# wengroup/matten

Hardware: AMD Instinct MI355X
Metric: edge_tensor_products_per_sec (higher is better)
Workload: dtype f32; 1 GPU; configs[2]: synthetic fcc-64 crystals (64 atoms, cutoff 5 A, 1152 edges each), paper hparams lmax=4, eval forward backbone+out_layer, one batch per step per GPU; last conv layer run for its live outputs only (258/842 radial-weight columns: the irreps its only reader takes) -- `value` counts 4 edge-TP per edge all the same, `value_full_layers` is the rate with the full last layer; nodes_per_gpu=64000, edges_per_gpu=1152000, conv_layers=4

## Files before the change

### include/matten_hip.h

```cpp
#ifndef MATTEN_HIP_H
#define MATTEN_HIP_H

#include <stddef.h>
#include <stdint.h>

#ifdef __cplusplus
extern "C" {
#endif

typedef void* matten_stream_t;

#define MATTEN_OK 0
#define MATTEN_EINVAL (-1)
#define MATTEN_ELAUNCH (-2)
#define MATTEN_ENOMEM (-3)

int matten_abi_version(void);

#define MATTEN_RADIAL_MAX_MID 3

size_t matten_csr_workspace_bytes(int64_t n_edges, int64_t n_nodes);
int matten_csr_counting_max_avg_degree(void);
int matten_csr_build(const int64_t* edge_index, int64_t n_edges, int64_t n_nodes, int32_t* perm,
                     int32_t* rowptr, int32_t* src_sorted, void* workspace, size_t workspace_bytes,
                     int32_t* err_flag, matten_stream_t stream);

int64_t matten_csr_split_bound(int64_t n_nodes, int64_t n_edges, int64_t max_len);
int matten_csr_split(const int32_t* rowptr, int64_t n_nodes, int64_t n_edges, int64_t max_len, int32_t* vrowptr,
                     int64_t* vseg, const float* num_neigh, float* vnn, matten_stream_t stream);

size_t matten_group_workspace_bytes(int64_t n, int64_t n_keys);
int matten_group_by_key(const int64_t* key, int64_t n, int64_t n_keys, int32_t* order, int32_t* seg,
                        void* workspace, size_t workspace_bytes, int32_t* err_flag, matten_stream_t stream);

int matten_species_embed(const int64_t* atomic_numbers, int64_t n_nodes, const int64_t* z_to_index,
                         int64_t min_z, int64_t max_z, int64_t n_species, const float* weight ,
                         const float* bias , int64_t dim, int64_t* species_index, int32_t* species_i32,
                         float* node_feats, float* node_attrs, int32_t* err_flag, matten_stream_t stream);

int matten_edge_geom(const float* pos, const int64_t* edge_index, const float* edge_cell_shift,
                     const float* cell, int64_t n_cells, const int64_t* batch, const int32_t* perm,
                     int64_t n_edges, int64_t n_nodes, int lmax, int n_basis, float r_start, float r_end,
                     float* geom_sorted, float* sh_sorted, int sh_stride, float* edge_vectors, float* edge_lengths,
                     float* edge_attrs, float* edge_embedding, matten_stream_t stream);
int matten_edge_geom_bwd(const float* geom_sorted, const float* dy, int64_t sh_stride, const float* dlen, int lmax,
                         int64_t n_edges, int64_t n_nodes, const int32_t* rowptr, const int32_t* out_ptr,
                         const int32_t* out_perm, const int32_t* perm, const float* edge_cell_shift, int64_t n_cells,
                         const int64_t* ptr, float* dv, float* dpos, float* dcell, matten_stream_t stream);

int matten_radial_mlp(const float* geom_sorted, int64_t n_edges, int n_basis, float r_start, float r_end,
                      const float* w0p, int nb_pad, const float* w1p, const float* w2p, int hidden, int w_pad,
                      float act_cst, void* w_edge, int out_is_bf16, matten_stream_t stream);
int matten_radial_mlp_deep(const float* geom_sorted, int64_t n_edges, int n_basis, float r_start, float r_end,
                           const float* w0p, int nb_pad, const float* w_mid, int n_mid, const float* w2p, int hidden,
                           int w_pad, float act_cst, void* w_edge, int out_is_bf16, matten_stream_t stream);

int matten_tp_tile_nodes(void);
int matten_tp_paths(const float* x, int64_t d_in, const void* w_edge, int64_t w_pad, const float* sh_sorted,
                    int64_t sh_dim, const int32_t* rowptr, const int32_t* src_sorted, int64_t n_nodes,
                    const int32_t* path_entries, const int32_t* unit_start, int64_t n_entries,
                    int64_t units_per_tile, int64_t d_mid, float avg_num_neighbors, const float* num_neigh,
                    float* agg , int w_is_bf16, matten_stream_t stream);

int matten_agg_linear_max_mt(void);
int matten_agg_linear_block_chunks(void);
size_t matten_agg_linear_lds_bytes(int64_t w_stride, int64_t n_io, int64_t n_blocks);
size_t matten_agg_linear_max_lds_bytes(void);
int matten_agg_linear(const float* agg, int64_t ld, const int32_t* order, const int32_t* seg, int64_t n_species,
                      const float* wtab, int64_t w_stride, const int32_t* io_table, int64_t n_io,
                      const int32_t* blocks, int64_t n_blocks, const float* add, int64_t add_ld, int64_t d_out,
                      int64_t n_rows, float* out, matten_stream_t stream);
int matten_agg_linear_gate(const float* agg, int64_t ld, const int32_t* order, const int32_t* seg, int64_t n_species,
                           const float* wtab, int64_t w_stride, const int32_t* io_table, int64_t n_io,
                           const int32_t* blocks, int64_t n_blocks, const float* add, int64_t add_ld, int64_t d_out,
                           int64_t n_rows, const int32_t* cmeta, const float* act_cst, const float* bn_scale,
                           const float* bn_shift, int64_t d_act, float* out, matten_stream_t stream);
int matten_agg_linear_gate_sets(void);
int matten_radial_hidden(const float* geom_sorted, int64_t n_edges, int n_basis, float r_start, float r_end,
                         const float* w0p, int nb_pad, const float* w1p, int hidden, uint16_t* h2s,
                         const float* h_scale, matten_stream_t stream);
int matten_radial_hidden_multi(const float* geom_sorted, int64_t n_edges, int n_basis, float r_start, float r_end,
                               const float* const* w0p, int nb_pad, const float* const* w1p, int hidden,
                               uint16_t* const* h2s, const float* const* h_scale, int n_layers,
                               matten_stream_t stream);
int matten_radial_hidden_deep(const float* geom_sorted, int64_t n_edges, int n_basis, float r_start, float r_end,
                              const float* w0p, int nb_pad, const float* w_mid, int n_mid, int hidden, uint16_t* h2s,
                              const float* h_scale, matten_stream_t stream);
int matten_radial_hidden_multi_deep(const float* geom_sorted, int64_t n_edges, int n_basis, float r_start, float r_end,
                                    const float* const* w0p, int nb_pad, const float* const* w_mid, int n_mid, int hidden,
                                    uint16_t* const* h2s, const float* const* h_scale, int n_layers,
                                    matten_stream_t stream);
int matten_tp_fused(const float* x, int64_t d_in, const uint16_t* h2s, const float* w2p, int64_t w_pad,
                    const float* sh_sorted, int64_t sh_stride, const int32_t* rowptr, const int32_t* src_sorted,
                    int64_t n_nodes, const int32_t* group_entries, const int32_t* unit_map, int64_t n_entries,
                    int64_t units_per_tile, int64_t lds_floats_per_wave, int64_t d_mid, float avg_num_neighbors,
                    const float* num_neigh, const uint16_t* a_split, const float* a_scale_inv,
                    float* agg , matten_stream_t stream);

int matten_tp_wreg(void);
int matten_tp_max_cols(void);
int matten_tp_max_cols_l0(void);
int matten_tp_max_cols_l1(void);
int matten_tp_groups_hash(void);

int matten_species_linear(const float* x, int64_t d_in, const int32_t* order, const int32_t* seg, int64_t n_species,
                          const float* wp, int64_t w_stride, const int32_t* segs, int64_t n_segs, int64_t d_out,
                          const float* add, int64_t add_ld, int64_t n_rows, float* out, matten_stream_t stream);

int matten_species_linear_rows(const float* x, int64_t d_in, const int32_t* order, const int32_t* seg, int64_t n_species,
                               const float* wp, int64_t w_stride, const int32_t* segs, int64_t n_segs, int64_t d_out,
                               const float* add, int64_t add_ld, int64_t n_rows, float* out, matten_stream_t stream);

int matten_species_linear_walk_all_blocks(void);
int64_t matten_species_linear_lds_w_floats(void);
int64_t matten_species_linear_rows_lds_bytes(void);

int matten_gate_bn(const float* x, int64_t d_in, const int32_t* meta, int64_t d_out, const float* act_cst,
                   const float* running_mean, const float* running_var, const float* bn_weight,
                   const float* bn_bias, float eps, int64_t n_rows, float* out, matten_stream_t stream);

int matten_segment_reduce(const float* x, int64_t dim, const int64_t* ptr, int64_t n_segments, int mean,
                          float* out, matten_stream_t stream);
int matten_segment_minmax(const float* x, int64_t dim, const int64_t* ptr, int64_t n_segments, int take_max, float* out,
                          int64_t* arg, matten_stream_t stream);
int matten_segment_minmax_bwd(const float* dy, int64_t dim, const int64_t* arg, int64_t n_segments, float* dx,
                              matten_stream_t stream);

int64_t matten_radial_mlp_bwd_small_slices(int64_t n_edges);
int64_t matten_radial_mlp_bwd_w2_ranges(int64_t n_edges, int64_t w_pad);
int matten_radial_mlp_bwd(const float* geom_sorted, int64_t n_edges, int n_basis, float r_start, float r_end,
                          const float* w0p, int nb_pad, const float* w1p, const float* w2p, int hidden, int w_pad,
                          int w_cols, const void* dw, int64_t dw_ld, int dw_is_bf16, float* h2_scratch,
                          float* part_small, float* part_w2, float scale0, float scale1, float scale2,
                          float* grad_small, float* grad_w2, matten_stream_t stream);
int64_t matten_radial_mlp_bwd_w2_ranges_deep(int64_t n_edges, int64_t w_pad, int n_mid);
int matten_radial_mlp_bwd_deep(const float* geom_sorted, int64_t n_edges, int n_basis, float r_start, float r_end,
                               const float* w0p, int nb_pad, const float* w_mid, int n_mid, const float* w2p, int hidden,
                               int w_pad, int w_cols, const void* dw, int64_t dw_ld, int dw_is_bf16, float* h2_scratch,
                               float* part_small, float* part_w2, float scale0, float scale1, float scale2,
                               float* grad_small, float* grad_w2, matten_stream_t stream);
int matten_radial_mlp_bwd_len(const float* geom_sorted, int64_t n_edges, int n_basis, float r_start, float r_end,
                              const float* w0p, int nb_pad, const float* w_mid, int n_mid, const float* w2p, int hidden,
                              int w_pad, int w_cols, const void* dw, int64_t dw_ld, int dw_is_bf16, float* dlen,
                              matten_stream_t stream);
int matten_radial_pack(const float* w0, const float* w1, const float* w2, int n_basis, int nb_pad, int w_cols, int w_pad,
                       float scale0, float scale1, float scale2, float* w0p, float* w1p, float* w2p,
                       matten_stream_t stream);
int matten_radial_pack_deep(const float* w0, const float* w_mid, int n_mid, const float* w2, int n_basis, int nb_pad,
                            int w_cols, int w_pad, float scale0, float scale1, float scale2, float* w0p, float* w_mid_p,
                            float* w2p, matten_stream_t stream);
int matten_radial_pack_cols(const float* w0, const float* w1, const float* w2, int n_basis, int nb_pad, int w_cols,
                            const int64_t* cols, int n_cols, int w_pad, float scale0, float scale1, float scale2, float* w0p,
                            float* w1p, float* w2p, matten_stream_t stream);
int matten_radial_h_scale(const float* w0, const float* w1, int n_basis, float r_start, float r_end, float act_cst,
                          float* out2, matten_stream_t stream);
int matten_radial_pack_cols_deep(const float* w0, const float* w_mid, int n_mid, const float* w2, int n_basis, int nb_pad,
                                 int w_cols, const int64_t* cols, int n_cols, int w_pad, float scale0, float scale1,
                                 float scale2, float* w0p, float* w_mid_p, float* w2p, matten_stream_t stream);
int matten_radial_h_scale_deep(const float* w0, const float* w_mid, int n_mid, int n_basis, float r_start, float r_end,
                               float act_cst, float* out2, matten_stream_t stream);
int matten_split_a_tiles(const float* w2p, int64_t w_pad, const int32_t* group_entries, int64_t n_entries,
                         const float* h_scale, uint16_t* frag, float* scale_inv, matten_stream_t stream);
int matten_gather_scale(const float* src, const int64_t* idx, const float* scale, int64_t n, int64_t scale_period,
                        int scale_by_source, float* out, const int64_t* perm2, float* out2, matten_stream_t stream);
int64_t matten_species_linear_wgrad_scratch_floats(int64_t n_rows, int64_t n_species, int64_t w_stride);

int matten_dense_rows(const float* x, int64_t n_in, const float* q, int64_t n_out, int64_t n_rows, float* out,
                      matten_stream_t stream);

int matten_elastic_props(const void* c, int is_fp64, int layout, int64_t n, double* voigt, double* compliance,
                         double* props, int32_t* flags, matten_stream_t stream);
int matten_elastic_props_bwd(const double* voigt, const double* compliance, const double* props, const int32_t* flags,
                             const double* g_props, const double* g_voigt, const double* g_compliance, int is_fp64,
                             int layout, int64_t n, void* g_c, matten_stream_t stream);
int matten_elastic_directional(const double* compliance, const int32_t* flags, const double* dirs, int64_t n,
                               int64_t n_dirs, double* young, double* beta, double* ext, int32_t* arg,
                               matten_stream_t stream);
int matten_elastic_pair(const double* compliance, const int32_t* flags, const double* dirs, const double* cos_sin,
                        int64_t n, int64_t n_dirs, int64_t n_angles, double* maps, double* ext, int32_t* arg,
                        matten_stream_t stream);
int matten_elastic_acoustic(const double* voigt, const int32_t* flags, const double* density, const double* dirs, int64_t n,
                            int64_t n_dirs, double modulus_unit, double* vel, double* ext, int32_t* arg, int32_t* n_unstable,
                            matten_stream_t stream);
int matten_elastic_directional_bwd(const double* compliance, const int32_t* flags, const double* dirs, int64_t n,
                                   int64_t n_dirs, const double* g_young, const double* g_beta, const double* g_ext,
                                   const int32_t* arg, double* g_compliance, matten_stream_t stream);
int matten_elastic_acoustic_bwd(const double* voigt, const int32_t* flags, const double* density, const double* dirs,
                                int64_t n, int64_t n_dirs, double modulus_unit, const double* g_vel, const double* g_ext,
                                const int32_t* arg, double* g_voigt, matten_stream_t stream);
int matten_elastic_refine(const double* compliance, const int32_t* flags, const double* dirs, const double* cos_sin,
                          const double* ext_dir, const int32_t* arg_dir, const double* ext_pair, const int32_t* arg_pair,
                          int64_t n, int64_t n_dirs, int64_t n_angles, double tol, int64_t max_iter, double* value,
                          double* vec_n, double* vec_m, int32_t* status, int32_t* iterations, matten_stream_t stream);

int matten_elastic_kelvin(const double* voigt, const int32_t* flags, int64_t n, double* moduli, double* vectors,
                          double* dilatation, matten_stream_t stream);
int matten_elastic_kelvin_bwd(const double* vectors, const int32_t* flags, const double* g_moduli, int64_t n,
                              double* g_voigt, matten_stream_t stream);
int matten_elastic_kelvin_clamp(const double* voigt, const double* moduli, const double* vectors, double floor, int64_t n,
                                double* out, matten_stream_t stream);

int matten_elastic_polycrystal(const double* voigt, const int32_t* flags, const double* moduli, const double* vectors,
                               int64_t n, int hs_grid, double sc_tol, int sc_max_iter, double* out, double* media,
                               int32_t* status, matten_stream_t stream);
int matten_elastic_polycrystal_bwd(const double* voigt, const int32_t* flags, const double* out, const int32_t* status,
                                   const double* g_sc, int64_t n, double* g_voigt, matten_stream_t stream);

int matten_rank2_props(const void* t, int is_fp64, int64_t n, double* vals, double* axes, double* props, int32_t* flags,
                       matten_stream_t stream);
int matten_rank2_props_bwd(const double* vals, const double* axes, const double* props, const int32_t* flags,
                           const double* g_vals, const double* g_props, int is_fp64, int64_t n, void* g_t,
                           matten_stream_t stream);

int matten_wigner_d(const double* R, int64_t G, int lmax, double orth_tol, double* D, int32_t* flags, matten_stream_t stream);
int matten_irreps_rotate(const void* x, int is_fp64, int64_t n, int64_t dim, const int32_t* layout, int K, const double* D,
                         const int32_t* flags, const int32_t* index, int64_t G, int transpose, void* out,
                         matten_stream_t stream);
int matten_irreps_average(const void* x, int is_fp64, int64_t n, int64_t dim, const int32_t* layout, int K, const double* D,
                          const int32_t* flags, int64_t G, const int64_t* op_ptr, const int32_t* op_idx,
                          const double* weights, int transpose, void* out, double* deviation, matten_stream_t stream);

#define MATTEN_SYM_MAX_OPS 48
#define MATTEN_SYM_MAX_ATOMS 1024
#define MATTEN_SYM_NOT_FINITE 1
#define MATTEN_SYM_RANGE 2
#define MATTEN_SYM_TOO_LARGE 4
#define MATTEN_SYM_AMBIGUOUS 8
#define MATTEN_SYM_TRUNC 16
#define MATTEN_SYM_NOT_PERIODIC 32
int matten_lattice_group(const double* cell, int64_t B, double symprec, int8_t* N_out, int32_t* n_lat, int32_t* flags,
                         matten_stream_t stream);
int matten_crystal_symmetry(const double* pos, const double* cell, const int64_t* Z, const int64_t* ptr, const uint8_t* pbc,
                            int64_t B, int64_t N_total, double symprec, int max_trans, const int8_t* N_in,
                            const int32_t* n_lat, const int32_t* lat_flags, double* rot, int8_t* rot_int, double* trans,
                            int32_t* n_rot, int32_t* src, int32_t* n_trans, double* ttrans, int32_t* tsrc, int32_t* flags,
                            matten_stream_t stream);
int matten_irreps_average_atoms(const void* x, int is_fp64, int64_t n, int64_t dim, const int32_t* layout, int K,
                                const double* D, const int32_t* flags, int64_t B, int64_t G_cap, const int32_t* n_ops,
                                const int32_t* row_struct, const int32_t* src, void* out, matten_stream_t stream);



int matten_tp_backward(const float* x, int64_t d_in, const void* w_edge, int64_t w_ld, const float* sh_sorted,
                       int64_t sh_stride, const int32_t* src_sorted, const int32_t* dst_sorted,
                       const int32_t* col_meta, int64_t n_cols, const uint8_t* nnz_ijk, const float* nnz_c,
                       const float* g_agg, int64_t d_mid, float avg_num_neighbors, const float* num_neigh,
                       int64_t n_edges, float* dx, void* dw, int64_t dw_ld, const int32_t* in_ptr,
                       const int32_t* in_cols, int64_t n_in, int edge_is_bf16 ,
                       matten_stream_t stream);

// ... 187 lines not shown
```

### matten_amd/_lib.py

```python
from __future__ import annotations

import ctypes
import os
from ctypes import c_float, c_int, c_int32, c_int64, c_size_t, c_void_p

_HERE = os.path.dirname(os.path.abspath(__file__))
LIB_PATH = os.path.join(_HERE, "libmatten_hip.so")

ABI_VERSION = 47

P = c_void_p
SIGNATURES = {
    "matten_abi_version": (c_int, []),
    "matten_csr_workspace_bytes": (c_size_t, [c_int64, c_int64]),
    "matten_group_workspace_bytes": (c_size_t, [c_int64, c_int64]),
    "matten_csr_counting_max_avg_degree": (c_int, []),
    "matten_csr_build": (c_int, [P, c_int64, c_int64, P, P, P, P, c_size_t, P, P]),
    "matten_csr_split_bound": (c_int64, [c_int64, c_int64, c_int64]),
    "matten_csr_split": (c_int, [P, c_int64, c_int64, c_int64, P, P, P, P, P]),
    "matten_group_by_key": (c_int, [P, c_int64, c_int64, P, P, P, c_size_t, P, P]),
    "matten_species_embed": (c_int, [P, c_int64, P, c_int64, c_int64, c_int64, P, P, c_int64, P, P, P, P, P, P]),
    "matten_edge_geom": (c_int, [P, P, P, P, c_int64, P, P, c_int64, c_int64, c_int, c_int, c_float, c_float, P, P, c_int, P, P, P, P, P]),
    "matten_radial_mlp": (c_int, [P, c_int64, c_int, c_float, c_float, P, c_int, P, P, c_int, c_int, c_float, P, c_int, P]),
    "matten_radial_mlp_deep": (c_int, [P, c_int64, c_int, c_float, c_float, P, c_int, P, c_int, P, c_int, c_int, c_float, P, c_int,
                                       P]),
    "matten_tp_tile_nodes": (c_int, []),
    "matten_tp_paths": (c_int, [P, c_int64, P, c_int64, P, c_int64, P, P, c_int64, P, P, c_int64, c_int64, c_int64, c_float, P, P, c_int,
                                P]),
    "matten_radial_hidden_multi": (c_int, [P, c_int64, c_int, c_float, c_float, P, c_int, P, c_int, P, P, c_int, P]),
    "matten_radial_hidden_multi_deep": (c_int, [P, c_int64, c_int, c_float, c_float, P, c_int, P, c_int, c_int, P, P, c_int, P]),
    "matten_agg_linear_max_mt": (c_int, []),
    "matten_agg_linear_block_chunks": (c_int, []),
    "matten_agg_linear_lds_bytes": (c_size_t, [c_int64, c_int64, c_int64]),
    "matten_agg_linear_max_lds_bytes": (c_size_t, []),
    "matten_agg_linear": (c_int, [P, c_int64, P, P, c_int64, P, c_int64, P, c_int64, P, c_int64, P, c_int64, c_int64,
                                  c_int64, P, P]),
    "matten_agg_linear_gate": (c_int, [P, c_int64, P, P, c_int64, P, c_int64, P, c_int64, P, c_int64, P, c_int64, c_int64,
                                       c_int64, P, P, P, P, c_int64, P, P]),
    "matten_agg_linear_gate_sets": (c_int, []),
    "matten_radial_hidden": (c_int, [P, c_int64, c_int, c_float, c_float, P, c_int, P, c_int, P, P, P]),
    "matten_radial_hidden_deep": (c_int, [P, c_int64, c_int, c_float, c_float, P, c_int, P, c_int, c_int, P, P, P]),
    "matten_tp_wreg": (c_int, []),
    "matten_tp_max_cols": (c_int, []),
    "matten_tp_max_cols_l0": (c_int, []),
    "matten_tp_max_cols_l1": (c_int, []),
    "matten_tp_groups_hash": (c_int, []),
    "matten_tp_fused": (c_int, [P, c_int64, P, P, c_int64, P, c_int64, P, P, c_int64, P, P, c_int64, c_int64, c_int64, c_int64, c_float, P, P, P, P, P]),
    "matten_species_linear": (c_int, [P, c_int64, P, P, c_int64, P, c_int64, P, c_int64, c_int64, P, c_int64, c_int64, P, P]),
    "matten_species_linear_rows": (c_int, [P, c_int64, P, P, c_int64, P, c_int64, P, c_int64, c_int64, P, c_int64, c_int64, P, P]),
    "matten_radial_mlp_bwd_small_slices": (c_int64, [c_int64]),
    "matten_radial_mlp_bwd_w2_ranges": (c_int64, [c_int64, c_int64]),
    "matten_radial_mlp_bwd_w2_ranges_deep": (c_int64, [c_int64, c_int64, c_int]),
    "matten_radial_mlp_bwd": (c_int, [P, c_int64, c_int, c_float, c_float, P, c_int, P, P, c_int, c_int, c_int, P, c_int64,
                                      c_int, P, P, P, c_float, c_float, c_float, P, P, P]),
    "matten_radial_mlp_bwd_deep": (c_int, [P, c_int64, c_int, c_float, c_float, P, c_int, P, c_int, P, c_int, c_int, c_int, P,
                                           c_int64, c_int, P, P, P, c_float, c_float, c_float, P, P, P]),
    "matten_radial_pack": (c_int, [P, P, P, c_int, c_int, c_int, c_int, c_float, c_float, c_float, P, P, P, P]),
    "matten_radial_pack_deep": (c_int, [P, P, c_int, P, c_int, c_int, c_int, c_int, c_float, c_float, c_float, P, P, P, P]),
    "matten_radial_pack_cols": (c_int, [P, P, P, c_int, c_int, c_int, P, c_int, c_int, c_float, c_float, c_float, P, P, P, P]),
    "matten_radial_pack_cols_deep": (c_int, [P, P, c_int, P, c_int, c_int, c_int, P, c_int, c_int, c_float, c_float, c_float, P, P,
                                             P, P]),
    "matten_radial_h_scale": (c_int, [P, P, c_int, c_float, c_float, c_float, P, P]),
    "matten_radial_h_scale_deep": (c_int, [P, P, c_int, c_int, c_float, c_float, c_float, P, P]),
    "matten_split_a_tiles": (c_int, [P, c_int64, P, c_int64, P, P, P, P]),
    "matten_gather_scale": (c_int, [P, P, P, c_int64, c_int64, c_int, P, P, P, P]),
    "matten_species_linear_walk_all_blocks": (c_int, []),
    "matten_species_linear_lds_w_floats": (c_int64, []),
    "matten_species_linear_rows_lds_bytes": (c_int64, []),
    "matten_species_linear_wgrad_scratch_floats": (c_int64, [c_int64, c_int64, c_int64]),
    "matten_tp_backward": (c_int, [P, c_int64, P, c_int64, P, c_int64, P, P, P, c_int64, P, P, P, c_int64, c_float, P, c_int64, P, P, c_int64,
                                   P, P, c_int64, c_int, P]),
    "matten_tp_backward_lit": (c_int, [P, c_int64, P, c_int64, P, c_int64, P, P, P, c_int64, c_int64, P, c_int64, P, c_int64, c_float,
                                       P, c_int64, P, P, c_int64, c_int, c_int64, P, P, P, c_int, P]),
    "matten_tp_backward_lit_wfree": (c_int, [P, c_int64, P, P, P, P, c_int64, P, P, P, c_int64, c_int64, P, c_int64, P, c_int64, c_float,
                                             P, c_int64, P, P, c_int64, c_int, c_int64, P, P, P, c_int64, c_int, c_int, P]),
    "matten_tp_backward_sh": (c_int, [P, c_int64, P, c_int64, P, P, P, c_int64, c_int64, P, c_int64, P, c_int64, c_float, P, c_int64,
                                      c_int, P, c_int64, c_int, P]),
    "matten_radial_mlp_bwd_len": (c_int, [P, c_int64, c_int, c_float, c_float, P, c_int, P, c_int, P, c_int, c_int, c_int, P,
                                          c_int64, c_int, P, P]),
    "matten_edge_geom_bwd": (c_int, [P, P, c_int64, P, c_int, c_int64, c_int64, P, P, P, P, P, c_int64, P, P, P, P, P]),
    "matten_adam_step": (c_int, [P, P, P, P, c_int64, P, c_float, c_float, c_float, c_float, c_float, P]),
    "matten_adam_ctl_workspace_bytes": (c_size_t, [c_int64]),
    "matten_adam_step_ctl": (c_int, [P, P, P, P, P, c_int64, P, P, P, P, c_size_t, c_float, c_float, c_float, c_float, c_float,
                                     c_float, c_int, c_int, P]),
    "matten_species_linear_wgrad": (c_int, [P, c_int64, P, c_int64, P, P, c_int64, c_int64, P, c_int64, c_int64, P, P, P]),
    "matten_gate_bwd": (c_int, [P, c_int64, P, c_int64, P, P, c_int64, P, P]),
    "matten_bn_scratch_floats": (c_int64, [c_int64, c_int64]),
    "matten_bn_train_fwd": (c_int, [P, c_int64, c_int64, P, P, c_int64, P, P, c_float, P, P, P, P, P, c_float, P, P]),
    "matten_bn_train_bwd": (c_int, [P, P, c_int64, c_int64, P, P, c_int64, P, P, P, c_float, P, P, P, P, P, P, P]),
    "matten_bn_train_fwd_valid": (c_int, [P, c_int64, c_int64, P, P, c_int64, P, P, c_float, P, P, P, P, P, c_float, P, P, P]),
    "matten_bn_train_bwd_valid": (c_int, [P, P, c_int64, c_int64, P, P, c_int64, P, P, P, c_float, P, P, P, P, P, P, P, P]),
    "matten_norm_act": (c_int, [P, c_int64, c_int64, P, c_int64, c_int, c_float, P, P, P, P, c_float, P, P]),
    "matten_norm_act_bwd": (c_int, [P, P, c_int64, c_int64, P, c_int64, c_int, c_float, P, P]),
    "matten_bn_eval_bwd_scratch_floats": (c_int64, [c_int64, c_int64]),
    "matten_gate_bn_eval_bwd": (c_int, [P, c_int64, P, c_int64, P, P, c_int64, P, P, P, c_float, P, c_int64, P, P, P, P, P]),
    "matten_norm_act_bn_eval_bwd": (c_int, [P, P, c_int64, c_int64, P, c_int64, c_int, c_float, P, P, P, c_float, P, P, P, P,
                                            P]),
    "matten_instance_norm_fwd": (c_int, [P, c_int64, c_int64, P, P, c_int64, P, P, c_int64, P, P, c_float, P, P, P, P]),
    "matten_instance_norm_bwd": (c_int, [P, P, c_int64, c_int64, P, P, c_int64, P, P, c_int64, P, P, P, c_float, P, P, P, P]),
    "matten_segment_reduce_bwd": (c_int, [P, c_int64, P, c_int64, c_int, P, P]),
    "matten_graph_prep": (c_int, [P, P, P, c_int64, ctypes.c_double, P, P, P, P, P, P]),
    "matten_graph_prep_pbc": (c_int, [P, P, P, P, c_int64, ctypes.c_double, P, P, P, P, P, P, P, P]),
    "matten_neighbor_rows_count": (c_int, [P, P, P, P, P, P, ctypes.c_double, c_int64, P, P]),
    "matten_neighbor_rows_fill": (c_int, [P, P, P, P, P, P, ctypes.c_double, c_int64, P, c_int64, P, P, P, P]),
    "matten_neighbor_cells_row_capacity": (c_int, []),
    "matten_neighbor_cells_max_axis_bins": (c_int, []),
    "matten_neighbor_cells_grid": (c_int, [P, P, P, P, P, P, c_int64, ctypes.c_double, P, P, P, P]),
    "matten_neighbor_cells_bin": (c_int, [P, P, P, P, P, P, c_int64, P, P, P]),
    "matten_neighbor_cells_scatter": (c_int, [P, P, P, P, c_int64, P, P, P]),
    "matten_neighbor_cells_count": (c_int, [P, P, P, P, P, P, P, P, P, P, P, ctypes.c_double, c_int64, P, P]),
    "matten_neighbor_cells_fill": (c_int, [P, P, P, P, P, P, P, P, P, P, P, ctypes.c_double, c_int64, P, c_int64, P, P, P, P]),
    "matten_neighbor_count": (c_int, [P, P, P, P, P, P, ctypes.c_double, c_int64, c_int64, P, P, P]),
    "matten_neighbor_summary": (c_int, [P, P, c_int64, P, P]),
    "matten_neighbor_fill": (c_int, [P, P, P, P, P, P, ctypes.c_double, c_int64, c_int64, P, c_int64, P, P, P, P, c_int64,
                                     P, P, P, P]),
    "matten_neighbor_scan": (c_int, [P, c_int64, P, P]),
    "matten_neighbor_fill_capped": (c_int, [P, P, P, P, P, P, ctypes.c_double, c_int64, c_int64, P, P, c_int64, P, c_int64,
                                            c_int64, c_int64, P, P, P, P, P, P, P, P, P]),
    "matten_gate_bn": (c_int, [P, c_int64, P, c_int64, P, P, P, P, P, c_float, c_int64, P, P]),
    "matten_segment_reduce": (c_int, [P, c_int64, P, c_int64, c_int, P, P]),
    "matten_segment_minmax": (c_int, [P, c_int64, P, c_int64, c_int, P, P, P]),
    "matten_segment_minmax_bwd": (c_int, [P, c_int64, P, c_int64, P, P]),
    "matten_dense_rows": (c_int, [P, c_int64, P, c_int64, c_int64, P, P]),
    "matten_elastic_props": (c_int, [P, c_int, c_int, c_int64, P, P, P, P, P]),
    "matten_elastic_props_bwd": (c_int, [P, P, P, P, P, P, P, c_int, c_int, c_int64, P, P]),
    "matten_elastic_directional": (c_int, [P, P, P, c_int64, c_int64, P, P, P, P, P]),
    "matten_elastic_pair": (c_int, [P, P, P, P, c_int64, c_int64, c_int64, P, P, P, P]),
    "matten_elastic_acoustic": (c_int, [P, P, P, P, c_int64, c_int64, ctypes.c_double, P, P, P, P, P]),
    "matten_elastic_directional_bwd": (c_int, [P, P, P, c_int64, c_int64, P, P, P, P, P, P]),
    "matten_elastic_acoustic_bwd": (c_int, [P, P, P, P, c_int64, c_int64, ctypes.c_double, P, P, P, P, P]),
    "matten_elastic_refine": (c_int, [P, P, P, P, P, P, P, P, c_int64, c_int64, c_int64, ctypes.c_double, c_int64, P, P, P, P, P,
                                      P]),
    "matten_elastic_kelvin": (c_int, [P, P, c_int64, P, P, P, P]),
    "matten_elastic_kelvin_bwd": (c_int, [P, P, P, c_int64, P, P]),
    "matten_elastic_kelvin_clamp": (c_int, [P, P, P, ctypes.c_double, c_int64, P, P]),
    "matten_elastic_polycrystal": (c_int, [P, P, P, P, c_int64, c_int, ctypes.c_double, c_int, P, P, P, P]),
    "matten_elastic_polycrystal_bwd": (c_int, [P, P, P, P, P, c_int64, P, P]),
    "matten_rank2_props": (c_int, [P, c_int, c_int64, P, P, P, P, P]),
    "matten_rank2_props_bwd": (c_int, [P, P, P, P, P, P, c_int, c_int64, P, P]),
    "matten_wigner_d": (c_int, [P, c_int64, c_int, ctypes.c_double, P, P, P]),
    "matten_irreps_rotate": (c_int, [P, c_int, c_int64, c_int64, P, c_int, P, P, P, c_int64, c_int, P, P]),
    "matten_irreps_average": (c_int, [P, c_int, c_int64, c_int64, P, c_int, P, P, c_int64, P, P, P, c_int, P, P, P]),
    "matten_lattice_group": (c_int, [P, c_int64, ctypes.c_double, P, P, P, P]),
    "matten_crystal_symmetry": (c_int, [P, P, P, P, P, c_int64, c_int64, ctypes.c_double, c_int, P, P, P, P, P, P, P, P, P, P, P,
                                        P, P]),
    "matten_irreps_average_atoms": (c_int, [P, c_int, c_int64, c_int64, P, c_int, P, P, c_int64, c_int64, P, P, P, P, P]),
    "matten_batch_gather_lds_rows": (c_int, []),
    "matten_batch_gather_max_streams": (c_int, []),
    "matten_batch_gather": (c_int, [P, c_int64, P, c_int64, c_int64, c_int64, P]),
    "matten_batch_gather_padded": (c_int, [P, c_int64, P, c_int64, c_int64, c_int64, c_int64, c_int64, c_int64, P, P]),
    "matten_selected_loss_tile_elems": (c_int, []),
    "matten_selected_loss_max_blocks": (c_int, []),
    "matten_selected_loss_workspace_bytes": (c_size_t, [c_int64, c_int64]),
    "matten_selected_loss": (c_int, [P, P, P, c_int64, c_int64, c_int, P, P, P, P, c_size_t, P]),
    "matten_selected_loss_bwd": (c_int, [P, P, P, c_int64, c_int64, c_int, P, P, P, P]),
    "matten_valid_loss_workspace_bytes": (c_size_t, [c_int64, c_int64]),
    "matten_valid_loss": (c_int, [P, P, P, c_int64, c_int64, c_int, P, P, P, P, c_size_t, P]),
    "matten_valid_loss_bwd": (c_int, [P, P, P, c_int64, c_int64, c_int, P, P, P, P]),
}

_lib = None


class MattenHipError(RuntimeError):
    pass


def load() -> ctypes.CDLL:
    global _lib
    if _lib is not None:
        return _lib
    if not os.path.exists(LIB_PATH):
        raise MattenHipError(
            f"{LIB_PATH} not found: the HIP extension is not built. matten_amd has no CPU fallback; "
            "run `make -C matten_amd/csrc` (needs hipcc, --offload-arch=gfx950)."
        )
    import torch

    lib = ctypes.CDLL(LIB_PATH)
    for name, (res, args) in SIGNATURES.items():
        try:
            fn = getattr(lib, name)
        except AttributeError as e:
            raise MattenHipError(f"symbol {name} missing from {LIB_PATH}") from e
        fn.restype = res
        fn.argtypes = args
    v = lib.matten_abi_version()
    if v != ABI_VERSION:
        raise MattenHipError(f"ABI version mismatch: library {v}, python binding {ABI_VERSION}")
    _lib = lib
    return lib


_ERRORS = {-1: "MATTEN_EINVAL (bad argument)", -2: "MATTEN_ELAUNCH (HIP launch failed)", -3: "MATTEN_ENOMEM (workspace too small)"}


def check(rc: int, what: str) -> None:
    if rc != 0:
        raise MattenHipError(f"{what} failed: {_ERRORS.get(rc, rc)}")
```

### matten_amd/csrc/tp_fused.hip

```cpp
#include "tp_walk.h"

namespace {

using namespace matten_walk;

constexpr int KIND_MERGED = 256;
constexpr int KIND_WREG = 512;
struct StoreAgg {
    template <class G>
    __device__ __forceinline__ void store(const Args& a, const GroupEntry& ge, const float* __restrict__ acc,
                                          float a_scale_inv, int node, int j, int u, bool valid) const {
        if (TPF_LAB_NO_STORE ? (valid && acc[0] == 12345.678f) : valid) {
            const float nn = a.avg_nn > 0.0f ? a.avg_nn : a.num_neigh[node];
            const float norm = nn > 0.0f ? a_scale_inv / sqrtf(nn) : 0.0f;
            float* orow = a.agg + (int64_t)node * a.d_mid;
            const bool merged = (ge.kind & KIND_MERGED) != 0;
            const GroupEntry& g2 = (&ge)[merged ? 1 : 0];
            const bool second = merged && u >= 2;
            const unsigned mask = merged ? (second ? g2.mask : (unsigned)g2.w_base) : ge.mask;
            const int uc = second ? u - 2 : u;
#pragma unroll
            for (int cc = 0; cc < G::NC; ++cc) {
                if ((mask >> cc) & 1u) {
                    const int d3 = 2 * G::L3[cc] + 1;
                    const int ks = second ? g2.t_off[cc] : ge.t_off[cc];
                    float* op = orow + (second ? g2.out_off[cc] : ge.out_off[cc]) + (ks ? uc : uc * d3);
                    const int kstep = ks ? ks : 1;
#pragma unroll
                    for (int k = 0; k < 2 * matten::CG_LMAX + 1; ++k)
                        if (k < d3) op[k * kstep] = acc[G::OFF[cc] + k] * norm;
                }
            }
        }
    }
};

template <int L1, int GI>
__device__ __forceinline__ void run_group(const Args& a, const GroupEntry& ge, float* __restrict__ tile, int node,
                                          int lane, bool valid, int beg, int deg_node, int maxdeg) {
    const int deg = valid ? deg_node : 0;
    using G = matten::Group<L1, GI>;
    constexpr int NC = G::NC;
    float acc[G::NACC];
#pragma unroll
    for (int k = 0; k < G::NACC; ++k) acc[k] = 0.0f;

    const unsigned mask = ge.mask;
    const int cu_log2 = ge.cu_log2;
    const int cu = 1 << cu_log2;
    const int npw = 64 >> cu_log2;
    const int ch_log2 = npw >= 16 ? 0 : (4 - (6 - cu_log2));
    const int CH = 1 << ch_log2;
    const int T = npw >= 16 ? (npw >> 4) : 1;
    const int ncols = ge.mul * NC;
    const int MT = (ncols + 15) >> 4;
    const int ycol = MT * 16;
    const int stride = MT * 16 + 32 + 4;

    const int j = lane >> cu_log2;
    const int u = lane & (cu - 1);
    const int g = lane >> 4, c = lane & 15;
    const int xcol = ge.x_off + u * G::D1;
    const bool cmajor = WregOk<L1, GI, 3>::value && (ge.kind & KIND_WREG) != 0;
    const int wcol0 = cmajor ? u : u * NC, wstep = cmajor ? cu : 1;
    constexpr int CAPC = cap_channels(L1, NC);
    constexpr int MTMAX = (CAPC * NC + 15) / 16;
    f16x8 ah[MTMAX], al[MTMAX];
    float a_scale_inv;
    {
        float av[MTMAX][8];
        float amax = 0.0f;
#pragma unroll
        for (int mt = 0; mt < MTMAX; ++mt) {
#pragma unroll
            for (int kk = 0; kk < 8; ++kk) {
                const int k = 16 * (kk >> 2) + 4 * g + (kk & 3);
                av[mt][kk] = (mt < MT) ? a.w2p[(int64_t)k * a.w_pad + ge.w_base + mt * 16 + c] : 0.0f;
                amax = fmaxf(amax, fabsf(av[mt][kk]));
            }
        }
#pragma unroll
        for (int off = 32; off > 0; off >>= 1) amax = fmaxf(amax, __shfl_xor(amax, off));
        int e = (int)((__float_as_uint(amax) >> 23) & 0xffu) - 127;
        e = amax > 0.0f ? max(-100, min(100, e)) : 13;
        const float a_scale = __uint_as_float((unsigned)(127 + 13 - e) << 23);
        a_scale_inv = __uint_as_float((unsigned)(127 - 13 + e) << 23);
#pragma unroll
        for (int mt = 0; mt < MTMAX; ++mt) {
#pragma unroll
            for (int kk = 0; kk < 8; ++kk) {
                _Float16 hi, lo;
                split_f16(av[mt][kk] * a_scale, hi, lo);
                ah[mt][kk] = hi;
                al[mt][kk] = lo;
            }
        }
    }

    const int e_last = deg > 0 ? beg + deg - 1 : 0;
    float xn[G::D1];
    int src_nn;
    {
        const int src0 = a.src_sorted[min(beg, e_last)];
        src_nn = a.src_sorted[min(beg + 1, e_last)];
        const float* xp0 = a.x + (int64_t)src0 * a.d_in + xcol;
#pragma unroll
        for (int i = 0; i < G::D1; ++i) xn[i] = xp0[i];
    }
    for (int s0 = 0; s0 < maxdeg; s0 += CH) {
#pragma unroll
        for (int t = 0; t < 4; ++t) {
            if (t < T) {
                const int n = 16 * t + c;
                const int jn = n >> ch_log2, so = n & (CH - 1);
                const int begn = __shfl(beg, jn << cu_log2);
                const int degn = __shfl(deg_node, jn << cu_log2);
                f16x8 bh = {0, 0, 0, 0, 0, 0, 0, 0}, bl = {0, 0, 0, 0, 0, 0, 0, 0};
                if (s0 + so < degn) {
                    const int64_t en = begn + s0 + so;
                    const f16x8* hp = reinterpret_cast<const f16x8*>(a.h2s + en * (2 * HID) + g * 8);
                    bh = hp[0];
                    bl = hp[HID / 8];
                    const f32x4* yp4 = reinterpret_cast<const f32x4*>(a.sh + en * a.sh_stride + g * 8);
                    f32x4* yd = reinterpret_cast<f32x4*>(tile + (16 * t + c) * stride + ycol + g * 8);
                    yd[0] = yp4[0];
                    yd[1] = yp4[1];
                }
#pragma unroll
                for (int mt = 0; mt < MTMAX; ++mt) {
                    if (mt < MT) {
                        const f32x4 zero = {0.f, 0.f, 0.f, 0.f};
                        f32x4 dx = __builtin_amdgcn_mfma_f32_16x16x32_f16(al[mt], bh, zero, 0, 0, 0);
                        f32x4 dh = __builtin_amdgcn_mfma_f32_16x16x32_f16(ah[mt], bh, zero, 0, 0, 0);
                        dx = __builtin_amdgcn_mfma_f32_16x16x32_f16(ah[mt], bl, dx, 0, 0, 0);
                        *reinterpret_cast<f32x4*>(tile + (16 * t + c) * stride + mt * 16 + 4 * g) =
                            dh + SPLIT_LO_INV * dx;
                    }
                }
            }
        }
        __builtin_amdgcn_s_waitcnt(0xc07f);
        __builtin_amdgcn_wave_barrier();
        for (int so = 0; so < CH; ++so) {
            const int s = s0 + so;
            if (s >= maxdeg) break;
            float x[G::D1];
#pragma unroll
            for (int i = 0; i < G::D1; ++i) x[i] = xn[i];
            {
                const float* xp = a.x + (int64_t)src_nn * a.d_in + xcol;
#pragma unroll
                for (int i = 0; i < G::D1; ++i) xn[i] = xp[i];
                src_nn = a.src_sorted[min(beg + s + 2, e_last)];
            }
            if (s < deg) {
                const float* wp = tile + ((j << ch_log2) + so) * stride + wcol0;
                const float* yp = tile + ((j << ch_log2) + so) * stride + ycol + G::Y0;
                float y[G::NY], w[NC];
#pragma unroll
                for (int jj = 0; jj < G::NY; ++jj) y[jj] = yp[jj];
#pragma unroll
                for (int cc = 0; cc < NC; ++cc) w[cc] = wp[cc * wstep];
                G::apply(mask, x, y, w, acc);
            }
        }
        __builtin_amdgcn_wave_barrier();
    }
    StoreAgg{}.store<G>(a, ge, acc, a_scale_inv, node, j, u, valid);
}

#define MATTEN_RGS_ARGS a, ge, tile, stage, (um >> 8) & 0xffff, tile_id, r, reps, lane, StoreAgg{}
#define MATTEN_RGS_WR(L1, GI, TT, TD, P, WR) \
    do { \
        using HM = HotMask<L1, GI>; \
        if (HM::M0 && ge.mask == HM::M0) run_group_shared<L1, GI, TT, TD, P, HM::M0, WR>(MATTEN_RGS_ARGS); \
        else if (HM::M1 && ge.mask == HM::M1) run_group_shared<L1, GI, TT, TD, P, HM::M1, WR>(MATTEN_RGS_ARGS); \
        else run_group_shared<L1, GI, TT, TD, P, 0u, WR>(MATTEN_RGS_ARGS); \
    } while (0)
template <int L1, int GI, int TT, int TD, bool P>
__device__ __forceinline__ void run_group_shared_any(const Args& a, const GroupEntry& ge, float* __restrict__ tile,
                                                     float* __restrict__ stage, int um, int tile_id, int r, int reps, int lane) {
    if constexpr (TT == 1 && WregOk<L1, GI, 4>::value) {
        if ((ge.kind & KIND_WREG) && ge.cu_log2 == 4) {
            MATTEN_RGS_WR(L1, GI, TT, TD, P, 4);
            return;
        }
    }
    if constexpr (TT == 1 && WregOk<L1, GI, 3>::value) {
        if ((ge.kind & KIND_WREG) && ge.cu_log2 == 3) {
            MATTEN_RGS_WR(L1, GI, TT, TD, P, 3);
            return;
        }
    }
    if (ge.kind & KIND_WREG) return;
    MATTEN_RGS_WR(L1, GI, TT, TD, P, 0);
}
#define MATTEN_RGS(L1, GI, TT, TD, P) run_group_shared_any<L1, GI, TT, TD, P>(a, ge, tile, stage, um, tile_id, r, reps, lane)
#if defined(MATTEN_LAB) && defined(TPF_ONLY_VARIANT)
#ifndef TPF_ONLY_MASK
#define TPF_ONLY_MASK 0
#endif
#ifndef TPF_ONLY_WR
#define TPF_ONLY_WR 0
#endif
#define MATTEN_RGS_ONLY(L1, GI, TT, TD, P) run_group_shared<L1, GI, TT, TD, P, (unsigned)(TPF_ONLY_MASK), (TT == 1 ? TPF_ONLY_WR : 0)>(MATTEN_RGS_ARGS)
#define MATTEN_GROUP_CASE_SHARED(L1, GI) \
    case (L1 * matten::GROUP_KIND_STRIDE + GI): \
        if (TPF_ONLY_VARIANT == 0) MATTEN_RGS_ONLY(L1, GI, 1, (TPF_CHUNK_DEEP && L1 == 0 ? 2 : 0), true); \
        else if (TPF_ONLY_VARIANT == 1) MATTEN_RGS_ONLY(L1, GI, 2, 0, false); \
        else if (TPF_ONLY_VARIANT == 2) MATTEN_RGS_ONLY(L1, GI, 1, (TPF_CHUNK_DEEP && L1 == 0 ? 2 : TwoDeepOk<L1, GI>::value ? 1 : 0), false); \
        else MATTEN_RGS_ONLY(L1, GI, 1, 0, false); \
        break;
#else
#define MATTEN_GROUP_CASE_SHARED(L1, GI) \
    case (L1 * matten::GROUP_KIND_STRIDE + GI): \
        if (paired && TPF_CHUNK_DEEP && L1 == 0 && nodes_per_wave <= 8 && nodes_per_wave >= 4) MATTEN_RGS(L1, GI, 1, (L1 == 0 ? 2 : 0), true); \
        else if (paired) MATTEN_RGS(L1, GI, 1, 0, true); \
        else if (nodes_per_wave > 16) MATTEN_RGS(L1, GI, 2, 0, false); \
        else if (TPF_CHUNK_DEEP && L1 == 0 && nodes_per_wave <= 8 && nodes_per_wave >= 4) MATTEN_RGS(L1, GI, 1, (L1 == 0 ? 2 : 0), false); \
        else if (TwoDeepOk<L1, GI>::value && nodes_per_wave <= 8 && nodes_per_wave >= TPF_TWO_DEEP_MIN_NPW) MATTEN_RGS(L1, GI, 1, (TwoDeepOk<L1, GI>::value ? 1 : 0), false); \
        else MATTEN_RGS(L1, GI, 1, 0, false); \
        break;
#endif

#define MATTEN_GROUP_CASE(L1, GI) \
    case (L1 * matten::GROUP_KIND_STRIDE + GI): run_group<L1, GI>(a, ge, tile, un.node, lane, un.valid, un.beg, un.deg, un.maxdeg); break;

#ifndef TPF_MIN_BLOCKS
#define TPF_MIN_BLOCKS 3
#endif
#ifndef TPF_CHUNK_DEEP
#define TPF_CHUNK_DEEP 1
#endif
#ifndef TPF_TWO_DEEP_MIN_NPW
#define TPF_TWO_DEEP_MIN_NPW 2
#endif
#if defined(MATTEN_LAB) && defined(TPF_ONLY_L1) && defined(TPF_ONLY_GI)
#define TPF_FOR_EACH_GROUP(X) X(TPF_ONLY_L1, TPF_ONLY_GI)
#elif defined(MATTEN_LAB) && defined(TPF_ONLY_LIGHT)
#define TPF_FOR_EACH_GROUP(X) X(0, 0) X(1, 0) X(1, 1)
#elif defined(MATTEN_LAB) && defined(TPF_ONLY_HEAVY)
#define TPF_FOR_EACH_GROUP(X) X(2, 0) X(2, 1) X(3, 0) X(3, 1) X(4, 0) X(4, 1)
#else
#define TPF_FOR_EACH_GROUP(X) MATTEN_FOR_EACH_GROUP(X)
#endif
__global__ __launch_bounds__(WAVES_PER_BLOCK * 64, TPF_MIN_BLOCKS) void tp_fused_kernel(Args a, const GroupEntry* __restrict__ entries,
                                                                        const int* __restrict__ umap,
                                                                        int n_entries, int units_per_tile,
                                                                        int blocks_per_tile, int n_tiles) {
    extern __shared__ __attribute__((aligned(16))) float lds[];
    const int xcd = blockIdx.x % N_XCD;
    const int q = blockIdx.x / N_XCD;
    const int tile_id = (q / blocks_per_tile) * N_XCD + xcd;
    if (tile_id >= n_tiles) return;
    const int wave = __builtin_amdgcn_readfirstlane(threadIdx.x >> 6);
    const int unit = (q % blocks_per_tile) * WAVES_PER_BLOCK + wave;
    if (unit >= units_per_tile) return;
    const int lane = threadIdx.x & 63;
    float* tile = lds + wave * a.lds_per_wave;

    const int um = __builtin_amdgcn_readfirstlane(umap[unit]);
    if (((um >> 8) & 0xffff) >= n_entries) return;
    const GroupEntry& ge = entries[(um >> 8) & 0xffff];
    const int r = um & 255;
    const bool shared_stage = (um >> 24) & 1;
    const int reps = 1 << ((um >> 27) & 3);

    const int cu_log2 = ge.cu_log2;
    const int nodes_per_wave = 64 >> cu_log2;
    if (shared_stage) {
        float* stage = lds + WAVES_PER_BLOCK * a.lds_per_wave;
        const bool paired = (um >> 26) & 1;
        if ((um >> 25) & 1) {
            if (paired) run_loader_only_paired(a, ge, stage, tile_id, r, reps, lane);
            else run_loader_only(a, ge, stage, tile_id, r, reps, lane);
            return;
        }
        switch (ge.kind & (KIND_MERGED - 1)) {
            TPF_FOR_EACH_GROUP(MATTEN_GROUP_CASE_SHARED)
            default: break;
        }
        return;
    }
#if !(defined(MATTEN_LAB) && defined(TPF_ONLY_VARIANT))
    const UnitNodes un = unit_nodes(a, ge, tile_id, r, lane);
    switch (ge.kind & (KIND_MERGED - 1)) {
        TPF_FOR_EACH_GROUP(MATTEN_GROUP_CASE)
        default: break;
    }
#endif
}

constexpr int NT = 4;
__device__ __forceinline__ float silu(float z) {
#if defined(MATTEN_LAB) && defined(RH_ABLATE_NO_SILU)
    return z * 0.5f;
#endif
    return z * __builtin_amdgcn_rcpf(1.0f + __builtin_amdgcn_exp2f(-1.4426950408889634f * z));
}

template <int KS0, int N_MID>
__global__ __launch_bounds__(256) void radial_hidden_kernel(const float4* __restrict__ geom, int64_t E, int n_basis,
                                                            float r_start, float r_end,
                                                            const float* __restrict__ w0p,
                                                            const float* __restrict__ w_mid, _Float16* __restrict__ h2s,
                                                            const float* __restrict__ h_scale) {
    const int lane = threadIdx.x & 63;
    const int wave = threadIdx.x >> 6;
    const int g = lane >> 4, c = lane & 15;
    const int64_t e0 = ((int64_t)blockIdx.x * 4 + wave) * (NT * 16);
    if (e0 >= E) return;
    const float hs = h_scale ? *h_scale : 1.0f;
    const float inv_c = 1.0f / (r_end - r_start);
    const float bes_pref = sqrtf(2.0f * inv_c) * sqrtf((float)n_basis);
    float a1[N_MID > 0 ? N_MID : 1][2][8];
#pragma unroll
    for (int m = 0; m < N_MID; ++m)
#pragma unroll
        for (int kk = 0; kk < 8; ++kk) {
            int k = 16 * (kk >> 2) + 4 * g + (kk & 3);
            a1[m][0][kk] = w_mid[m * HID * HID + k * HID + c];
// ... 124 lines not shown
            }
#pragma unroll
            for (int r = 0; r < 4; ++r) {
                h0[r] = silu(h0[r]);
                h1[r] = silu(h1[r]);
            }
#pragma unroll
            for (int m = 0; m < N_MID; ++m) {
                f32x4 o0 = {0.f, 0.f, 0.f, 0.f}, o1 = {0.f, 0.f, 0.f, 0.f};
#pragma unroll
                for (int kk = 0; kk < 8; ++kk) {
                    const float b = kk < 4 ? h0[kk & 3] : h1[kk & 3];
                    o0 = __builtin_amdgcn_mfma_f32_16x16x4f32(a1[m][0][kk], b, o0, 0, 0, 0);
                    o1 = __builtin_amdgcn_mfma_f32_16x16x4f32(a1[m][1][kk], b, o1, 0, 0, 0);
                }
#pragma unroll
                for (int r = 0; r < 4; ++r) {
                    o0[r] = silu(o0[r]);
                    o1[r] = silu(o1[r]);
                }
                h0 = o0, h1 = o1;
            }
            if (e < E) {
                f16x8 hi, lo;
#pragma unroll
                for (int r = 0; r < 4; ++r) {
                    _Float16 h, ll;
                    split_f16(h0[r] * hs, h, ll);
                    hi[r] = h, lo[r] = ll;
                    split_f16(h1[r] * hs, h, ll);
                    hi[4 + r] = h, lo[4 + r] = ll;
                }
                f16x8* dst = reinterpret_cast<f16x8*>(h2s + e * (2 * HID) + g * 8);
                dst[0] = hi;
                dst[HID / 8] = lo;
            }
        }
    }
}

}

static int radial_hidden_multi_launch(const float* geom_sorted, int64_t n_edges, int n_basis, float r_start, float r_end,
                                      const float* const* w0p, int nb_pad, const float* const* w_mid, int n_mid, int hidden,
                                      uint16_t* const* h2s, const float* const* h_scale, int n_layers,
                                      matten_stream_t stream_) {
    hipStream_t stream = (hipStream_t)stream_;
    if (n_edges < 0 || hidden != HID || (nb_pad & 3) || nb_pad < n_basis || nb_pad > 16 || n_layers < 1 ||
        n_layers > RH_MAX_LAYERS || n_mid < 0 || n_mid > MATTEN_RADIAL_MAX_MID)
        return MATTEN_EINVAL;
    if (n_edges == 0) return MATTEN_OK;
    if (!geom_sorted || !w0p || (n_mid > 0 && !w_mid) || !h2s) return MATTEN_EINVAL;
    RadialLayers L{};
    L.n_layers = n_layers;
    for (int l = 0; l < n_layers; ++l) {
        if (!w0p[l] || (n_mid > 0 && !w_mid[l]) || !h2s[l]) return MATTEN_EINVAL;
        L.w0p[l] = w0p[l], L.w_mid[l] = n_mid > 0 ? w_mid[l] : nullptr, L.h2s[l] = (_Float16*)h2s[l];
        L.h_scale[l] = h_scale ? h_scale[l] : nullptr;
    }
    unsigned grid = (unsigned)matten_cdiv(n_edges, 4 * NT * 16);
#define LAUNCH(K, M) \
    radial_hidden_multi_kernel<K, M><<<grid, 256, 0, stream>>>((const float4*)geom_sorted, n_edges, n_basis, r_start, r_end, L)
#define LAUNCH_M(K)                  \
    switch (n_mid) {                 \
        case 0: LAUNCH(K, 0); break; \
        case 1: LAUNCH(K, 1); break; \
        case 2: LAUNCH(K, 2); break; \
        default: LAUNCH(K, 3); break; \
    }
    switch (nb_pad >> 2) {
        case 1: LAUNCH_M(1); break;
        case 2: LAUNCH_M(2); break;
        case 3: LAUNCH_M(3); break;
        default: LAUNCH_M(4); break;
    }
#undef LAUNCH_M
#undef LAUNCH
    MATTEN_LAUNCH_CHECK();
    return MATTEN_OK;
}

extern "C" int matten_radial_hidden_multi(const float* geom_sorted, int64_t n_edges, int n_basis, float r_start,
                                          float r_end, const float* const* w0p, int nb_pad, const float* const* w1p,
                                          int hidden, uint16_t* const* h2s, const float* const* h_scale, int n_layers,
                                          matten_stream_t stream_) {
    if (!w1p && n_edges > 0) return MATTEN_EINVAL;
    return radial_hidden_multi_launch(geom_sorted, n_edges, n_basis, r_start, r_end, w0p, nb_pad, w1p, 1, hidden, h2s,
                                      h_scale, n_layers, stream_);
}

extern "C" int matten_radial_hidden_multi_deep(const float* geom_sorted, int64_t n_edges, int n_basis, float r_start,
                                               float r_end, const float* const* w0p, int nb_pad, const float* const* w_mid,
                                               int n_mid, int hidden, uint16_t* const* h2s, const float* const* h_scale,
                                               int n_layers, matten_stream_t stream_) {
    return radial_hidden_multi_launch(geom_sorted, n_edges, n_basis, r_start, r_end, w0p, nb_pad, w_mid, n_mid, hidden, h2s,
                                      h_scale, n_layers, stream_);
}

static int radial_hidden_launch(const float* geom_sorted, int64_t n_edges, int n_basis, float r_start, float r_end,
                                const float* w0p, int nb_pad, const float* w_mid, int n_mid, int hidden, uint16_t* h2s,
                                const float* h_scale, matten_stream_t stream_) {
    hipStream_t stream = (hipStream_t)stream_;
    if (n_edges < 0 || hidden != HID || (nb_pad & 3) || nb_pad < n_basis || nb_pad > 16 || n_mid < 0 ||
        n_mid > MATTEN_RADIAL_MAX_MID)
        return MATTEN_EINVAL;
    if (n_edges == 0) return MATTEN_OK;
    if (!geom_sorted || !w0p || (n_mid > 0 && !w_mid) || !h2s) return MATTEN_EINVAL;
    unsigned grid = (unsigned)matten_cdiv(n_edges, 4 * NT * 16);
#define LAUNCH(K, M) \
    radial_hidden_kernel<K, M><<<grid, 256, 0, stream>>>((const float4*)geom_sorted, n_edges, n_basis, r_start, r_end, w0p, w_mid, (_Float16*)h2s, h_scale)
#define LAUNCH_M(K)                  \
    switch (n_mid) {                 \
        case 0: LAUNCH(K, 0); break; \
        case 1: LAUNCH(K, 1); break; \
        case 2: LAUNCH(K, 2); break; \
        default: LAUNCH(K, 3); break; \
    }
    switch (nb_pad >> 2) {
        case 1: LAUNCH_M(1); break;
        case 2: LAUNCH_M(2); break;
        case 3: LAUNCH_M(3); break;
        default: LAUNCH_M(4); break;
    }
#undef LAUNCH_M
#undef LAUNCH
    MATTEN_LAUNCH_CHECK();
    return MATTEN_OK;
}

extern "C" int matten_radial_hidden(const float* geom_sorted, int64_t n_edges, int n_basis, float r_start, float r_end,
                                    const float* w0p, int nb_pad, const float* w1p, int hidden, uint16_t* h2s,
                                    const float* h_scale, matten_stream_t stream_) {
    if (!w1p && n_edges > 0) return MATTEN_EINVAL;
    return radial_hidden_launch(geom_sorted, n_edges, n_basis, r_start, r_end, w0p, nb_pad, w1p, 1, hidden, h2s, h_scale,
                                stream_);
}

extern "C" int matten_radial_hidden_deep(const float* geom_sorted, int64_t n_edges, int n_basis, float r_start, float r_end,
                                         const float* w0p, int nb_pad, const float* w_mid, int n_mid, int hidden,
                                         uint16_t* h2s, const float* h_scale, matten_stream_t stream_) {
    return radial_hidden_launch(geom_sorted, n_edges, n_basis, r_start, r_end, w0p, nb_pad, w_mid, n_mid, hidden, h2s,
                                h_scale, stream_);
}

#if TPF_TRACING
static unsigned* g_tp_trace = nullptr;
static int64_t g_tp_trace_waves = 0, g_tp_trace_skip = 0;
extern "C" int matten_lab_tp_trace(unsigned* buf, int64_t n_waves, int64_t skip) {
    g_tp_trace = buf, g_tp_trace_waves = n_waves, g_tp_trace_skip = skip;
    return 0;
}
#endif

extern "C" int matten_tp_fused(const float* x, int64_t d_in, const uint16_t* h2s, const float* w2p, int64_t w_pad,
                               const float* sh_sorted, int64_t sh_stride, const int32_t* rowptr,
                               const int32_t* src_sorted, int64_t n_nodes, const int32_t* group_entries,
                               const int32_t* unit_map, int64_t n_entries, int64_t units_per_tile,
                               int64_t lds_floats_per_wave, int64_t d_mid, float avg_num_neighbors,
                               const float* num_neigh, const uint16_t* a_split, const float* a_scale_inv, float* agg,
                               matten_stream_t stream_) {
    hipStream_t stream = (hipStream_t)stream_;
    if (n_nodes < 0 || d_in <= 0 || w_pad <= 0 || sh_stride < 32 || (sh_stride & 3) || n_entries <= 0 ||
        units_per_tile <= 0 || d_mid <= 0 || lds_floats_per_wave <= 0 || (lds_floats_per_wave & 3))
        return MATTEN_EINVAL;
    if (n_nodes == 0) return MATTEN_OK;
    if (!x || !h2s || !w2p || !sh_sorted || !rowptr || !src_sorted || !group_entries || !unit_map || !agg)
        return MATTEN_EINVAL;
    if (!(avg_num_neighbors > 0.0f) && !num_neigh) return MATTEN_EINVAL;
    const size_t lds = sizeof(float) * ((size_t)lds_floats_per_wave * WAVES_PER_BLOCK + STAGE_TOTAL_FLOATS + PAIR_INFO_INTS);
    if (lds > 64 * 1024) return MATTEN_EINVAL;
    if ((a_split == nullptr) != (a_scale_inv == nullptr)) return MATTEN_EINVAL;
    Args a{x, (const _Float16*)h2s, w2p, (const _Float16*)a_split, a_scale_inv, sh_sorted, rowptr, src_sorted, num_neigh, agg, (int)d_in, (int)w_pad, (int)sh_stride,
           (int)d_mid, (int)n_nodes, (int)lds_floats_per_wave, avg_num_neighbors};
    const int n_tiles = (int)matten_cdiv(n_nodes, TILE_NODES);
    const int blocks_per_tile = (int)matten_cdiv(units_per_tile, WAVES_PER_BLOCK);
    const int64_t grid = matten_cdiv(n_tiles, N_XCD) * N_XCD * (int64_t)blocks_per_tile;
    if (grid >= ((int64_t)1 << 31)) return MATTEN_EINVAL;
#if TPF_TRACING
    a.trace = nullptr;
    if (g_tp_trace && grid * WAVES_PER_BLOCK <= g_tp_trace_waves) {
        if (g_tp_trace_skip <= 0) a.trace = g_tp_trace;
        if (g_tp_trace_skip == 0) g_tp_trace = nullptr;
        if (g_tp_trace_skip > 0) --g_tp_trace_skip;
    }
#endif
    tp_fused_kernel<<<(unsigned)grid, WAVES_PER_BLOCK * 64, lds, stream>>>(
        a, (const GroupEntry*)group_entries, unit_map, (int)n_entries, (int)units_per_tile, blocks_per_tile, n_tiles);
    MATTEN_LAUNCH_CHECK();
    return MATTEN_OK;
}

extern "C" int matten_tp_wreg(void) { return TPF_WREG ? TPF_WREG_MAX_L1 + 1 : 0; }
extern "C" int matten_tp_max_cols(void) { return TPF_MAX_COLS; }
extern "C" int matten_tp_max_cols_l0(void) { return TPF_MAX_COLS_L0; }
extern "C" int matten_tp_max_cols_l1(void) { return TPF_MAX_COLS_L1; }
extern "C" int matten_tp_groups_hash(void) { return matten::GROUPS_HASH; }
```

### matten_amd/csrc/tp_walk.h

```cpp
#pragma once
#include <type_traits>

#include "cg_gen.h"
#include "common.h"
#include "sh.h"

#ifndef MATTEN_LAB
#if defined(MATTEN_ABLATE_NO_GATHER) || defined(MATTEN_ABLATE_NO_XLOAD) || defined(MATTEN_ABLATE_NO_H2LOAD) || \
    defined(MATTEN_ABLATE_NO_MFMA) || defined(MATTEN_ABLATE_NO_VALU) || defined(MATTEN_ABLATE_NO_STORE) ||      \
    defined(MATTEN_ABLATE_NO_BARRIER) || defined(MATTEN_ABLATE_NO_LOOP) || defined(MATTEN_ABLATE_NO_EPI) || defined(MATTEN_ABLATE_ONE_YQUAD)
#error "MATTEN_ABLATE_* switches are honoured by -DMATTEN_LAB builds only (tools/*.sh)"
#endif
#endif
#if defined(MATTEN_LAB) && defined(MATTEN_ABLATE_NO_GATHER)
#define TPF_SRC(v) ((v) >= 0 ? (node < a.n_nodes ? node : 0) : 0)
#else
#define TPF_SRC(v) (v)
#endif
#if defined(MATTEN_LAB) && defined(MATTEN_ABLATE_NO_XLOAD)
#define TPF_XLD(xp, i, v) (1e-9f * (float)((v) + (i)))
#else
#define TPF_XLD(xp, i, v) ((xp)[i])
#endif
#if defined(MATTEN_LAB) && defined(MATTEN_ABLATE_NO_H2LOAD)
constexpr bool TPF_LAB_NO_H2LOAD = true;
#else
constexpr bool TPF_LAB_NO_H2LOAD = false;
#endif
#if defined(MATTEN_LAB) && defined(MATTEN_ABLATE_NO_MFMA)
constexpr bool TPF_LAB_NO_MFMA = true;
#else
constexpr bool TPF_LAB_NO_MFMA = false;
#endif
#if defined(MATTEN_LAB) && defined(MATTEN_ABLATE_NO_VALU)
constexpr bool TPF_LAB_NO_VALU = true;
#else
constexpr bool TPF_LAB_NO_VALU = false;
#endif
#if defined(MATTEN_LAB) && defined(MATTEN_ABLATE_NO_STORE)
constexpr bool TPF_LAB_NO_STORE = true;
#else
constexpr bool TPF_LAB_NO_STORE = false;
#endif
#if defined(MATTEN_LAB) && defined(MATTEN_ABLATE_NO_BARRIER)
constexpr bool TPF_LAB_NO_BARRIER = true;
#else
constexpr bool TPF_LAB_NO_BARRIER = false;
#endif
#if defined(MATTEN_LAB) && defined(MATTEN_ABLATE_NO_LOOP)
constexpr bool TPF_LAB_NO_LOOP = true;
#else
constexpr bool TPF_LAB_NO_LOOP = false;
#endif

#if defined(MATTEN_LAB) && defined(TPF_TRACE)
#define TPF_TRACING 1
#else
#define TPF_TRACING 0
#endif

namespace matten_walk {

#if TPF_TRACING
__device__ __forceinline__ unsigned tpf_stamp() {
    unsigned long long t;
    asm volatile("s_waitcnt lgkmcnt(0)\n\ts_memtime %0\n\ts_waitcnt lgkmcnt(0)" : "=s"(t) : : "memory");
    return (unsigned)t;
}
__device__ __forceinline__ unsigned tpf_stamp_hi() {
    unsigned long long t;
    asm volatile("s_waitcnt lgkmcnt(0)\n\ts_memtime %0\n\ts_waitcnt lgkmcnt(0)" : "=s"(t) : : "memory");
    return (unsigned)(t >> 32);
}
template <int N>
__device__ __forceinline__ unsigned tpf_stamp_after(float (&acc)[N]) {
    unsigned long long t;
    asm volatile("s_waitcnt lgkmcnt(0)\n\ts_memtime %0\n\ts_waitcnt lgkmcnt(0)"
                 : "=s"(t), "+v"(acc[0]), "+v"(acc[N / 2]), "+v"(acc[N - 1]) : : "memory");
    return (unsigned)t;
}
#endif

typedef float f32x4 __attribute__((ext_vector_type(4)));
typedef _Float16 f16x8 __attribute__((ext_vector_type(8)));

constexpr float SPLIT_LO_SCALE = 2048.0f;
constexpr float SPLIT_LO_INV = 1.0f / 2048.0f;
constexpr float F16_MIN_NORMAL = 6.103515625e-05f;

__device__ __forceinline__ void split_f16(float v, _Float16& hi, _Float16& lo) {
    const float h = fabsf(v) < F16_MIN_NORMAL ? 0.0f : (float)(_Float16)v;
    const float r = (v - h) * SPLIT_LO_SCALE;
    hi = (_Float16)h;
    lo = fabsf(r) < F16_MIN_NORMAL ? (_Float16)0.0f : (_Float16)r;
}

#ifndef TPF_SETPRIO
#define TPF_SETPRIO 3
#endif
#ifndef TPF_W_FIRST
#define TPF_W_FIRST 1
#endif
#ifndef TPF_W_FIRST2
#define TPF_W_FIRST2 1
#endif
#ifndef TPF_PAIR_SUM
#define TPF_PAIR_SUM 1
#endif
#ifndef TPF_EXACT_Y0
#define TPF_EXACT_Y0 0
#endif

#ifndef TPF_WREG
#define TPF_WREG 1
#endif
#ifndef TPF_WREG_ALO_LDS_MT
#define TPF_WREG_ALO_LDS_MT 5
#endif
#ifndef TPF_WREG_MAX_L1
#define TPF_WREG_MAX_L1 1
#endif

#ifndef TPF_REP_PREFETCH
#define TPF_REP_PREFETCH 1
#endif
#ifndef TPF_MAX_COLS
#define TPF_MAX_COLS 64
#endif
#ifndef TPF_MAX_COLS_L0
#define TPF_MAX_COLS_L0 96
#endif
#ifndef TPF_MAX_COLS_L1
#define TPF_MAX_COLS_L1 TPF_MAX_COLS
#endif
__host__ __device__ constexpr int cap_channels(int l1, int nc) {
    int cap = 64;
    while (cap > 1 && cap * nc > (l1 == 0 ? TPF_MAX_COLS_L0 : l1 == 1 ? TPF_MAX_COLS_L1 : TPF_MAX_COLS)) cap /= 2;
    return cap;
}
constexpr int TILE_NODES = 64;
constexpr int WAVES_PER_BLOCK = 4;
constexpr int N_XCD = 8;
constexpr int MAXC = matten::GROUP_MAX_COMBOS;
constexpr int HID = 32;

struct GroupEntry {
    int kind;
    int x_off;
    int mul;
    int cu_log2;
    unsigned mask;
    int w_base;
    int a_tile;
    int n_mt;
    int t_off[MAXC];
    int out_off[MAXC];
};
static_assert(sizeof(GroupEntry) == 32 * 4, "GroupEntry layout");

struct Args {
    const float* x;
    const _Float16* h2s;
    const float* w2p;
    const _Float16* a_split;
    const float* a_scale_inv;
    const float* sh;
    const int* rowptr;
    const int* src_sorted;
    const float* num_neigh;
    float* agg;
    int d_in, w_pad, sh_stride, d_mid, n_nodes, lds_per_wave;
    float avg_nn;
#if TPF_TRACING
    unsigned* trace;
#endif
};


struct UnitNodes {
    int node, beg, deg, maxdeg;
    bool valid;
};
struct RawNodes {
    int node, b0, b1;
    bool valid;
};
__device__ __forceinline__ RawNodes unit_nodes_issue(const Args& a, const GroupEntry& ge, int tile_id, int r, int lane) {
    const int cu_log2 = ge.cu_log2;
    const int nodes_per_wave = 64 >> cu_log2;
    const int g_in_tile = r * nodes_per_wave + (lane >> cu_log2);
    const int u = lane & ((1 << cu_log2) - 1);
    RawNodes n;
    n.node = tile_id * TILE_NODES + g_in_tile;
    const bool in_range = (g_in_tile < TILE_NODES) && (n.node < a.n_nodes);
    n.valid = in_range && (u < ge.mul);
    n.b0 = 0, n.b1 = 0;
    if (in_range) {
        n.b0 = a.rowptr[n.node];
        n.b1 = a.rowptr[n.node + 1];
    }
    return n;
}
__device__ __forceinline__ UnitNodes unit_nodes_finish(const RawNodes& raw) {
    UnitNodes n;
    n.node = raw.node, n.valid = raw.valid, n.beg = raw.b0, n.deg = raw.b1 - raw.b0;
    int maxdeg = n.deg;
#pragma unroll
    for (int off = 32; off > 0; off >>= 1) maxdeg = max(maxdeg, __shfl_xor(maxdeg, off));
    if constexpr (TPF_LAB_NO_LOOP) maxdeg = 0;
    n.maxdeg = maxdeg;
    return n;
}
__device__ __forceinline__ UnitNodes unit_nodes(const Args& a, const GroupEntry& ge, int tile_id, int r, int lane) {
    return unit_nodes_finish(unit_nodes_issue(a, ge, tile_id, r, lane));
}

constexpr int STAGE_ROW = 68;
constexpr int STAGE_TMAX = 2;
constexpr int STAGE_FLOATS = 16 * STAGE_TMAX * STAGE_ROW;
constexpr int STAGE_TOTAL_FLOATS = 2 * STAGE_FLOATS;

__device__ __forceinline__ const char* stage_safe_row(const Args& a) {
    return reinterpret_cast<const char*>(a.w2p + ((max(a.w_pad, 4) - 4) & ~3));
}

template <int MTC>
__device__ __forceinline__ void mfma_tiles(const f16x8* __restrict__ ah, const f16x8* __restrict__ al, f16x8 bh, f16x8 bl,
                                           float* __restrict__ trow) {
    const f32x4 zero = {0.f, 0.f, 0.f, 0.f};
    f32x4 dx[MTC], dh[MTC];
#pragma unroll
    for (int mt = 0; mt < MTC; ++mt) {
        dx[mt] = __builtin_amdgcn_mfma_f32_16x16x32_f16(al[mt], bh, zero, 0, 0, 0);
        dh[mt] = __builtin_amdgcn_mfma_f32_16x16x32_f16(ah[mt], bh, zero, 0, 0, 0);
    }
#pragma unroll
    for (int mt = 0; mt < MTC; ++mt) dx[mt] = __builtin_amdgcn_mfma_f32_16x16x32_f16(ah[mt], bl, dx[mt], 0, 0, 0);
#pragma unroll
    for (int mt = 0; mt < MTC; ++mt) *reinterpret_cast<f32x4*>(trow + mt * 16) = dh[mt] + SPLIT_LO_INV * dx[mt];
}



template <int TT>
struct StageLoader {
    const char* base;
    const char* safe;
    int64_t row_bytes;
    float* st_w;
    int beg_ld[TT], deg_ld[TT], so_ld[TT];
    int CH;
    f32x4 pf[TT];

    __device__ __forceinline__ void init(const Args& a, float* stage, int cu_log2, int beg, int deg_node) {
        const int npw = 64 >> cu_log2;
        const int ch_log2 = npw >= 16 ? 0 : 4 - (6 - cu_log2);
        CH = 1 << ch_log2;
        const int piece = threadIdx.x & 15;
        base = piece < 8 ? reinterpret_cast<const char*>(a.h2s) + piece * 16
                         : reinterpret_cast<const char*>(a.sh) + (piece - 8) * 16;
        row_bytes = piece < 8 ? (int64_t)(2 * HID * sizeof(_Float16)) : (int64_t)a.sh_stride * 4;
        safe = stage_safe_row(a);
        st_w = stage + (threadIdx.x >> 4) * STAGE_ROW + piece * 4;
#pragma unroll
        for (int t = 0; t < TT; ++t) {
            const int n = (int)(threadIdx.x >> 4) + 16 * t;
            const int jn = (n >> ch_log2) & (npw - 1);
            so_ld[t] = n & (CH - 1);
            beg_ld[t] = __shfl(beg, jn << cu_log2);
            deg_ld[t] = __shfl(deg_node, jn << cu_log2);
            pf[t] = f32x4{0.f, 0.f, 0.f, 0.f};
        }
    }
    __device__ __forceinline__ void issue(int s0) {
        if constexpr (TPF_LAB_NO_H2LOAD) return;
#pragma unroll
        for (int t = 0; t < TT; ++t)
            pf[t] = *reinterpret_cast<const f32x4*>(
                deg_ld[t] > 0 ? base + (int64_t)(beg_ld[t] + min(s0 + so_ld[t], deg_ld[t] - 1)) * row_bytes : safe);
    }
    __device__ __forceinline__ void publish(int buf) {
#pragma unroll
        for (int t = 0; t < TT; ++t)
            *reinterpret_cast<f32x4*>(st_w + buf * (16 * TT * STAGE_ROW) + 16 * t * STAGE_ROW) = pf[t];
    }
};

constexpr int PAIR_INFO_INTS = 2 * 16 * 2 + 2;
struct PairLoader {
    const char* base;
    const char* safe;
    int64_t row_bytes;
    float* st_w;
    int beg_ld[2], deg_ld[2], so_ld;
    int CH, maxdeg;
    f32x4 pf[2];

    __device__ __forceinline__ void init(const Args& a, float* stage, int* info, int cu_log2, int beg, int deg_node,
                                         int my_maxdeg) {
        const int npw = 64 >> cu_log2;
        const int ch_log2 = 4 - (6 - cu_log2);
        CH = 1 << ch_log2;
        const int wave = threadIdx.x >> 6, lane = threadIdx.x & 63;
        if ((wave & 1) == 0 && (lane & ((1 << cu_log2) - 1)) == 0) {
            info[((wave >> 1) * 16 + (lane >> cu_log2)) * 2] = beg;
            info[((wave >> 1) * 16 + (lane >> cu_log2)) * 2 + 1] = deg_node;
            if (lane == 0) info[2 * 16 * 2 + (wave >> 1)] = my_maxdeg;
        }
        __syncthreads();
        maxdeg = max(info[2 * 16 * 2], info[2 * 16 * 2 + 1]);
        const int piece = threadIdx.x & 15;
        base = piece < 8 ? reinterpret_cast<const char*>(a.h2s) + piece * 16
                         : reinterpret_cast<const char*>(a.sh) + (piece - 8) * 16;
        row_bytes = piece < 8 ? (int64_t)(2 * HID * sizeof(_Float16)) : (int64_t)a.sh_stride * 4;
        safe = stage_safe_row(a);
        const int n = (int)(threadIdx.x >> 4);
        st_w = stage + n * STAGE_ROW + piece * 4;
        const int jn = (n >> ch_log2) & (npw - 1);
        so_ld = n & (CH - 1);
#pragma unroll
        for (int t = 0; t < 2; ++t) {
            beg_ld[t] = info[(t * 16 + jn) * 2];
            deg_ld[t] = info[(t * 16 + jn) * 2 + 1];
            pf[t] = f32x4{0.f, 0.f, 0.f, 0.f};
        }
// ... 357 lines not shown
#pragma unroll
                    for (int cc = 0; cc < NC; ++cc) w[cc] = wp[cc];
                    asm volatile("" ::: "memory");
                }
                constexpr int Q0 = G::Y0 / 4 * 4, NQ = (G::Y0 + G::NY - Q0 + 3) / 4;
                float yq[4 * NQ];
                const f32x4* y4 = reinterpret_cast<const f32x4*>(yp - (G::Y0 - Q0));
#pragma unroll
                for (int q = 0; q < NQ; ++q) {
                    const f32x4 v = y4[q];
                    yq[4 * q] = v[0], yq[4 * q + 1] = v[1], yq[4 * q + 2] = v[2], yq[4 * q + 3] = v[3];
                }
#pragma unroll
                for (int jj = 0; jj < G::NY; ++jj) y[jj] = yq[G::Y0 - Q0 + jj];
                if constexpr (!WR && !TPF_W_FIRST2) {
#pragma unroll
                    for (int cc = 0; cc < NC; ++cc) w[cc] = wp[cc];
                }
            };
            auto pair_pass = [&](auto so_c) {
                const int so = so_c;
                const int s = s0 + so;
                float ya[G::NY], wa[NC], yb[G::NY], wb[NC], xa[G::D1], xc[G::D1];
                fetch(so_c, ya, wa);
                fetch(slot_next(so_c), yb, wb);
#pragma unroll
                for (int i = 0; i < G::D1; ++i) xa[i] = s < deg ? xn[i] : 0.0f, xc[i] = s + 1 < deg ? xb[i] : 0.0f;
                {
                    const float* xp = a.x + (int64_t)TPF_SRC(src_nn) * a.d_in + xcol;
#pragma unroll
                    for (int i = 0; i < G::D1; ++i) xn[i] = TPF_XLD(xp, i, src_nn);
                    src_nn = a.src_sorted[min(beg + s + 4, e_last)];
                }
                {
                    const float* xp = a.x + (int64_t)TPF_SRC(src_b) * a.d_in + xcol;
#pragma unroll
                    for (int i = 0; i < G::D1; ++i) xb[i] = TPF_XLD(xp, i, src_b);
                    src_b = a.src_sorted[min(beg + s + 5, e_last)];
                }
                G::apply2(CMASK ? CMASK : mask, xa, ya, wa, xc, yb, wb, acc);
            };
            if constexpr (WR) for_slots<0, WCH, 2>(pair_pass);
            else for (int so = 0; so < CH; so += 2) pair_pass(so);
        } else if constexpr (chunk_deep) {
#pragma unroll
            for (int i = 0; i < XQ; ++i) {
                const float* xp = a.x + (int64_t)TPF_SRC(sq[i]) * a.d_in + xcol;
                xnext[i] = TPF_XLD(xp, 0, sq[i]);
            }
#pragma unroll
            for (int i = 0; i < XQ; ++i) sq[i] = a.src_sorted[min(beg + s0 + 2 * CH + i, e_last)];
            if constexpr (WR) {
                for_slots<0, WCH, 1>([&](auto so_c) {
                    if (s0 + so_c < deg) contract(so_c, xcur + so_c);
                });
            } else {
#pragma unroll
                for (int so = 0; so < XQ; ++so) {
                    if (so < CH && s0 + so < deg) contract(so, xcur + so);
                }
            }
        } else if (two_deep) {
            auto pair_steps = [&](auto so_c) {
                const int so = so_c;
                const int s = s0 + so;
                if (s < deg) contract(so_c, xn);
                {
                    const float* xp = a.x + (int64_t)TPF_SRC(src_nn) * a.d_in + xcol;
#pragma unroll
                    for (int i = 0; i < G::D1; ++i) xn[i] = TPF_XLD(xp, i, src_nn);
                    src_nn = a.src_sorted[min(beg + s + 4, e_last)];
                }
                if (s + 1 < deg) contract(slot_next(so_c), xb);
                {
                    const float* xp = a.x + (int64_t)TPF_SRC(src_b) * a.d_in + xcol;
#pragma unroll
                    for (int i = 0; i < G::D1; ++i) xb[i] = TPF_XLD(xp, i, src_b);
                    src_b = a.src_sorted[min(beg + s + 5, e_last)];
                }
            };
            if constexpr (WR) for_slots<0, WCH, 2>(pair_steps);
            else for (int so = 0; so < CH; so += 2) pair_steps(so);
        } else if constexpr (WR != 0) {
            bool go = true;
            for_slots<0, WCH, 1>([&](auto so_c) {
                const int s = s0 + so_c;
                go = go && s < maxdeg;
                if (!go) return;
                float x[G::D1];
#pragma unroll
                for (int i = 0; i < G::D1; ++i) x[i] = xn[i];
                {
                    const float* xp = a.x + (int64_t)TPF_SRC(src_nn) * a.d_in + xcol;
#pragma unroll
                    for (int i = 0; i < G::D1; ++i) xn[i] = TPF_XLD(xp, i, src_nn);
                    src_nn = a.src_sorted[min(beg + s + 2, e_last)];
                }
                if (s < deg) contract(so_c, x);
            });
        } else {
            for (int so = 0; so < CH; ++so) {
                const int s = s0 + so;
                if (s >= maxdeg) break;
                float x[G::D1];
#pragma unroll
                for (int i = 0; i < G::D1; ++i) x[i] = xn[i];
                {
                    const float* xp = a.x + (int64_t)TPF_SRC(src_nn) * a.d_in + xcol;
#pragma unroll
                    for (int i = 0; i < G::D1; ++i) xn[i] = TPF_XLD(xp, i, src_nn);
                    src_nn = a.src_sorted[min(beg + s + 2, e_last)];
                }
                if (s < deg) contract(so, x);
            }
        }
#if TPF_TRACING
        const unsigned tr_c = tpf_stamp_after(acc);
#endif
        ld.publish(buf ^ 1);
#if TPF_TRACING
        const unsigned tr_d = tpf_stamp();
#endif
        if constexpr (TPF_LAB_NO_BARRIER) {
            __builtin_amdgcn_s_waitcnt(0xc07f);
            __builtin_amdgcn_wave_barrier();
        } else {
            __syncthreads();
        }
#if TPF_TRACING
        const unsigned tr_e = tpf_stamp();
        tr_mfma += (unsigned)(tr_b - tr_a), tr_con += (unsigned)(tr_c - tr_b), tr_pub += (unsigned)(tr_d - tr_c);
        tr_bar += (unsigned)(tr_e - tr_d), tr_chunks += 1;
        tr_a = tr_e;
#endif
    };
    if constexpr (chunk_deep) {
        for (int s0 = 0; s0 < maxdeg; s0 += 2 * CH) {
            chunk_body(s0, 0, xqa, xqb);
            if (s0 + CH < maxdeg) chunk_body(s0 + CH, 1, xqb, xqa);
        }
    } else {
        int buf = 0;
        for (int s0 = 0; s0 < maxdeg; s0 += CH, buf ^= 1) chunk_body(s0, buf, xqa, xqb);
    }
#if TPF_TRACING
    const unsigned tr_end = tpf_stamp();
#endif
    const int node_done = node;
    const bool valid_done = valid;
    if (TPF_REP_PREFETCH && more) start_group(unit_nodes_finish(raw_next));
#if TPF_TRACING
    tr_epi_sg += (unsigned)(tpf_stamp() - tr_end);
#endif
    epi.template store<G>(a, ge, acc, a_scale_inv, node_done, j, u, valid_done);
    if (!TPF_REP_PREFETCH && more) start_group(unit_nodes_finish(raw_next));
#if TPF_TRACING
    if (a.trace && lane == 0) {
        if (rep + 1 == reps) asm volatile("s_waitcnt vmcnt(0)" ::: "memory");
        const unsigned tr_out = tpf_stamp();
        tr_epi += (unsigned)(tr_out - tr_end);
        if (rep + 1 == reps) {
            unsigned* tr = a.trace + ((size_t)blockIdx.x * WAVES_PER_BLOCK + (threadIdx.x >> 6)) * 16;
            tr[0] = 1u, tr[1] = (unsigned)ge.kind, tr[2] = (unsigned)cu_log2 | (PAIRED ? 256u : 0u) | ((unsigned)reps << 9) | ((unsigned)TT << 12) | ((unsigned)MT << 16);
            tr[3] = tr_chunks, tr[4] = tr_pro, tr[5] = tr_mfma, tr[6] = tr_con, tr[7] = tr_pub, tr[8] = tr_bar;
            tr[9] = tr_epi, tr[10] = (unsigned)(tr_out - tr_in), tr[11] = (unsigned)ge.mask;
            tr[12] = tr_in, tr[13] = tr_in_hi, tr[14] = tr_pro_pre, tr[15] = tr_epi_sg;
        }
    }
#endif
    }
}

template <int L1, int GI> struct HotMask { static constexpr unsigned M0 = 0, M1 = 0; };
#ifndef TPF_NO_HOT_MASKS
template <> struct HotMask<0, 0> { static constexpr unsigned M0 = 0x1f, M1 = 0xf; };
#endif
#ifndef TPF_HOT_ALL
#define TPF_HOT_ALL 1
#endif
#if TPF_HOT_ALL
template <> struct HotMask<1, 0> { static constexpr unsigned M0 = 0x7f, M1 = 0; };
template <> struct HotMask<1, 1> { static constexpr unsigned M0 = 0x1b, M1 = 0xf; };
template <> struct HotMask<2, 0> { static constexpr unsigned M0 = 0x7ff, M1 = 0x6ff; };
template <> struct HotMask<2, 1> { static constexpr unsigned M0 = 0x1d, M1 = 0xf; };
template <> struct HotMask<3, 0> { static constexpr unsigned M0 = 0x3ff, M1 = 0x37f; };
template <> struct HotMask<3, 1> { static constexpr unsigned M0 = 0x7f, M1 = 0x3f; };
template <> struct HotMask<4, 0> { static constexpr unsigned M0 = 0xfb, M1 = 0; };
template <> struct HotMask<4, 1> { static constexpr unsigned M0 = 0x7d, M1 = 0; };
#endif
#ifndef TPF_HOT_ALT
#define TPF_HOT_ALT 1
#endif
#if TPF_HOT_ALT
template <> struct HotMask<0, 1> { static constexpr unsigned M0 = 0x7, M1 = 0; };
template <> struct HotMask<1, 4> { static constexpr unsigned M0 = 0x3f, M1 = 0; };
template <> struct HotMask<2, 4> { static constexpr unsigned M0 = 0x3f, M1 = 0; };
template <> struct HotMask<1, 2> { static constexpr unsigned M0 = 0xf, M1 = 0; };
template <> struct HotMask<1, 3> { static constexpr unsigned M0 = 0x3, M1 = 0; };
template <> struct HotMask<2, 2> { static constexpr unsigned M0 = 0x7, M1 = 0; };
template <> struct HotMask<2, 3> { static constexpr unsigned M0 = 0x3f, M1 = 0; };
template <> struct HotMask<3, 2> { static constexpr unsigned M0 = 0x1f, M1 = 0; };
template <> struct HotMask<3, 3> { static constexpr unsigned M0 = 0xf, M1 = 0; };
template <> struct HotMask<4, 2> { static constexpr unsigned M0 = 0x7, M1 = 0; };
template <> struct HotMask<4, 3> { static constexpr unsigned M0 = 0x3f, M1 = 0; };
#endif

}
```

### matten_amd/nn/conv.py

```python
from typing import Dict

import torch

import numpy as np

from .. import autograd as _ag
from .. import ops
from ..data.irreps import DataKey, ModuleIrreps
from ..o3 import Irreps
from ._tables import DerivedWeight, DeviceTables, WeightSlice
from .utils import ActivationLayer, NormalizationLayer, SpeciesLinear, UVUTensorProduct


import os as _os

GATE_APPLIED = "_amd_gate_applied"
GATE_FUSE = _os.environ.get("MATTEN_GATE_FUSE", "1") != "0"
KEPT_ONLY = "_amd_kept_irreps_only"
DEAD_PATH_ELIMINATION = _os.environ.get("MATTEN_DEAD_PATH_ELIMINATION", "1") != "0"
AGG_KM_MIN_ROWS = int(_os.environ.get("MATTEN_AGG_KM_MIN_ROWS", "8192"))


def _geometry(data) -> tuple:
    return data.get(DataKey.AMD_GEOM), data.get(DataKey.AMD_SH)


class PointConv(ModuleIrreps, torch.nn.Module):
    def __init__(
        self,
        irreps_in: Dict[str, Irreps],
        conv_layer_irreps: Irreps,
        fc_num_hidden_layers: int = 1,
        fc_hidden_size: int = 8,
        avg_num_neighbors: int = None,
    ):
        super().__init__()
        self.avg_num_neighbors = avg_num_neighbors
        self.init_irreps(irreps_in)
        self.__dict__["_ctor"] = dict(irreps_in=dict(irreps_in), fc_num_hidden_layers=fc_num_hidden_layers,
                                      fc_hidden_size=fc_hidden_size, avg_num_neighbors=avg_num_neighbors)
        self.__dict__["_view"] = None
        feats_in = self.irreps_in[DataKey.NODE_FEATURES]
        n_species = self.irreps_in[DataKey.NODE_ATTRS].dim
        edge_attrs = self.irreps_in[DataKey.EDGE_ATTRS]
        conv_layer_irreps = Irreps(conv_layer_irreps)

        self.lin1 = SpeciesLinear(feats_in, n_species, feats_in)
        self.tp = UVUTensorProduct(
            feats_in,
            edge_attrs,
            conv_layer_irreps,
            mlp_input_size=self.irreps_in[DataKey.EDGE_EMBEDDING].dim,
            mlp_hidden_size=fc_hidden_size,
            mlp_num_hidden_layers=fc_num_hidden_layers,
            mlp_activation="silu",
        )
        self.lin2 = SpeciesLinear(self.tp.irreps_out, n_species, conv_layer_irreps)
        self.sc = SpeciesLinear(feats_in, n_species, conv_layer_irreps)
        self.irreps_out[DataKey.NODE_FEATURES] = conv_layer_irreps
        self._lin1_sc = None
        self._lin1_sc_packed = DerivedWeight(self._pack_lin1_sc)
        from .. import plan as _plan
        import os
        self.agg_plan = None
        if self.tp.impl == "fused" and os.environ.get("MATTEN_AGG_LAYOUT", "km") == "km":
            ap = _plan.plan_agg_linear(self.tp.plan, n_species, conv_layer_irreps)
            if ap is not None and self._agg_fits(ap):
                self.agg_plan = ap
                self._agg_tables = DeviceTables(entries=ap.entries, io=ap.io_table, blocks=ap.blocks, gather=ap.gather,
                                                scale=ap.scale)
                self._agg_wtab = DerivedWeight(self._pack_agg_weights)

    def _pack_lin1_sc(self, w1: torch.Tensor, w2: torch.Tensor) -> torch.Tensor:
        return torch.cat([self.lin1._pack(w1), self.sc._pack(w2)], dim=1).contiguous()

    def _fused_lin1_sc_tables(self):
        if self._lin1_sc is None:
            p1, p2 = self.lin1.plan, self.sc.plan
            if len(p1.passes) != 1 or len(p2.passes) != 1 or not (p1.fully_covered and p2.fully_covered):
                self._lin1_sc = False
            else:
                seg2 = p2.passes[0].copy()
                seg2[:, 3] += p1.w_stride
                seg2[:, 5] += p1.d_out
                segs = np.concatenate([p1.passes[0], seg2])
                segs = segs[np.argsort(segs[:, 0], kind="stable")]
                self._lin1_sc = DeviceTables(meta=segs)
        return self._lin1_sc

    @staticmethod
    def _agg_fits(ap) -> bool:
        from .. import _lib
        try:
            lib = _lib.load()
        except Exception:
            return 4 * ap.w_stride <= 40 * 1024
        return lib.matten_agg_linear_lds_bytes(ap.w_stride, len(ap.io_table), len(ap.blocks)) <= lib.matten_agg_linear_max_lds_bytes()

    def _pack_agg_weights(self, w: torch.Tensor) -> torch.Tensor:
        t, dev = self._agg_tables, w.device
        gather, scale = t.get("gather", dev), t.get("scale", dev)
        return torch.where(gather >= 0, w[gather.clamp(min=0)] * scale[None, :], w.new_zeros(())).contiguous()

    def build_inference_view(self, kept_irreps) -> bool:
        kept = Irreps(kept_irreps).simplify()
        full_out = self.sc.irreps_out
        if any(sum(1 for _, ir2 in irr if ir2 == ir) != 1 for irr in (full_out, self.lin2.irreps_in) for _, ir in irr):
            return False
        if any(sum(1 for m2, ir2 in full_out if ir2 == ir and m2 == m) != 1 for m, ir in kept) or kept.dim >= full_out.dim:
            return False
        try:
            v = PointConv(conv_layer_irreps=kept, **self._ctor)
        except Exception:
            return False

        from .. import plan as _plan

        m_sc, m_l2 = _plan.linear_flat_submap(v.sc.plan, self.sc.plan), _plan.linear_flat_submap(v.lin2.plan, self.lin2.plan)
        fullp = {(q.i_in1, q.i_sh, q.l3, q.p3): q for q in self.tp.plan.paths}
        cols = []
        for q in v.tp.plan.paths:
            f = fullp.get((q.i_in1, q.i_sh, q.l3, q.p3))
            if f is None or f.mul != q.mul:
                return False
            cols.append(np.arange(f.w_off, f.w_off + f.mul))
        if m_sc is None or m_l2 is None or not cols:
            return False
        v.lin1 = self.lin1
        mlp, full = v.tp.weight_nn, self.tp.weight_nn
        last = len(full.hs) - 2
        for i in range(last):
            setattr(mlp, f"layer{i}", getattr(full, f"layer{i}"))
        mlp.__dict__["_hidden_from"] = full
        for mod in (v.sc, v.lin2, getattr(mlp, f"layer{last}")):
            del mod._parameters["weight"]
        v.__dict__["_slices"] = (WeightSlice(m_sc), WeightSlice(m_l2), WeightSlice(np.concatenate(cols), dim=1))
        self.__dict__["_view"] = v
        return True

    def _view_forward(self, data, differentiable: bool):
        v = self._view
        s_sc, s_l2, s_w2 = v._slices
        pick = (lambda sl, w: sl.select(w)) if differentiable else (lambda sl, w: sl.get(w))
        last = f"layer{len(self.tp.weight_nn.hs) - 2}"
        targets = ((v.sc, s_sc, self.sc.weight), (v.lin2, s_l2, self.lin2.weight),
                   (getattr(v.tp.weight_nn, last), s_w2, getattr(self.tp.weight_nn, last).weight))
        for mod, sl, w in targets:
            mod.__dict__["weight"] = pick(sl, w)
        try:
            return v(data)
        finally:
            if differentiable:
                for mod, _, _ in targets:
                    mod.__dict__["weight"] = None

    def forward(self, data: DataKey.Type) -> DataKey.Type:
        if self._view is not None and DEAD_PATH_ELIMINATION:
            data = self._view_forward(data, _ag.needs_grad_lazy(lambda: (data[DataKey.NODE_FEATURES], *_geometry(data),
                                                                         *_ag.params_of(self))))
            data[KEPT_ONLY] = True
            return data
        data.pop(KEPT_ONLY, None)
        x = data[DataKey.NODE_FEATURES]
        species = data[DataKey.AMD_SPECIES]
        fused = None if _ag.needs_grad(x, self.lin1.weight, self.sc.weight) else self._fused_lin1_sc_tables()
        if fused:
            wp = self._lin1_sc_packed.get(self.lin1.weight, self.sc.weight)
            d1, d2 = self.lin1.plan.d_out, self.sc.plan.d_out
            both = ops.species_linear(x, species, wp, self.lin1.plan.w_stride + self.sc.plan.w_stride,
                                      [fused.get("meta", x.device)], d1 + d2)
            x1, self_connection = both[:, :d1], both[:, d1:]
        else:
            self_connection = self.sc(x, species)
            x1 = self.lin1(x, species)
        if (self.agg_plan is not None and x1.shape[0] >= AGG_KM_MIN_ROWS
                and not _ag.needs_grad_lazy(lambda: (x1, self_connection, self.lin2.weight, *_geometry(data),
                                                     *_ag.params_of(self.tp.weight_nn)))):
            ap, t, dev = self.agg_plan, self._agg_tables, x1.device
            agg = self.tp(x1, data, self.avg_num_neighbors, out_layout=(t.get("entries", dev), ap.ld))
            gate = self.__dict__.get("_gate_fuse")
            if gate is not None:
                cmeta, act_cst, d_act, bn_scale, bn_shift = gate
                data[DataKey.NODE_FEATURES] = ops.agg_linear_gate(
                    agg, species, self._agg_wtab.get(self.lin2.weight), t.get("io", dev), t.get("blocks", dev), ap.d_out,
                    cmeta, act_cst, d_act, add=self_connection, bn_scale=bn_scale, bn_shift=bn_shift)
                data[GATE_APPLIED] = True
                return data
            data[DataKey.NODE_FEATURES] = ops.agg_linear(agg, species, self._agg_wtab.get(self.lin2.weight),
                                                         t.get("io", dev), t.get("blocks", dev), ap.d_out,
                                                         add=self_connection)
            return data
        agg = self.tp(x1, data, self.avg_num_neighbors)
        data[DataKey.NODE_FEATURES] = self.lin2(agg, species, add=self_connection)
        return data


class PointConvWithActivation(ModuleIrreps, torch.nn.Module):
    def __init__(
        self,
        irreps_in: Dict[str, Irreps],
        conv_layer_irreps: Irreps,
        fc_num_hidden_layers: int = 1,
        fc_hidden_size: int = 8,
        avg_num_neighbors: int = None,
        activation_type: str = "gate",
        activation_scalars: Dict[str, str] = {"e": "silu", "o": "tanh"},
        activation_gates: Dict[str, str] = {"e": "sigmoid", "o": "tanh"},
        normalization: str = None,
    ):
        super().__init__()
        self.init_irreps(irreps_in)
        self.act = ActivationLayer(
            self.irreps_in[DataKey.NODE_FEATURES],
            self.irreps_in[DataKey.EDGE_ATTRS],
            Irreps(conv_layer_irreps),
            activation_type=activation_type,
            activation_scalars=activation_scalars,
            activation_gates=activation_gates,
        )
        self.conv = PointConv(
            irreps_in=self.irreps_in,
            conv_layer_irreps=self.act.irreps_in,
            fc_num_hidden_layers=fc_num_hidden_layers,
            fc_hidden_size=fc_hidden_size,
            avg_num_neighbors=avg_num_neighbors,
        )
        self.norm = NormalizationLayer(self.act.irreps_out, method=normalization)
        self.irreps_out[DataKey.NODE_FEATURES] = self.act.irreps_out

    def _gate_fuse_args(self, dev):
        if not GATE_FUSE or self.conv.agg_plan is None or getattr(self.act, "activation_type", "gate") != "gate":
            return None
        if self.norm.method not in ("batch", "none", None):
            return None
        bn = self.norm.n
        if bn is not None and bn.training:
            return None
        fuse = self.__dict__.get("_fuse_tables")
        if fuse is None:
            from .. import plan as _plan

            cm = _plan.plan_agg_gate(self.conv.agg_plan, self.act.plan)
            fuse = False if cm is None else DeviceTables(cmeta=cm)
            self.__dict__["_fuse_tables"] = fuse
            self.__dict__["_fuse_bn"] = DerivedWeight(self._fold_bn)
        if fuse is False:
            return None
        scale = shift = None
        if bn is not None:
            scale, shift = self._fuse_bn.get(bn.running_mean, bn.running_var, bn.weight, bn.bias)
        return (fuse.get("cmeta", dev), self.act._tables.get("act_cst", dev), self.act.plan.irreps_out.dim, scale, shift)

    def _fold_bn(self, rm, rv, w, b):
        meta = torch.as_tensor(np.asarray(self.act.plan.meta).reshape(-1, 4)[:, 3].astype(np.int64), device=w.device)
        bn_idx, mean_idx = meta & 0xFFFF, (meta >> 16) & 0xFFFF
        scale = (w / torch.sqrt(rv + self.norm.n.eps))[bn_idx]
        has_mean = mean_idx != 0xFFFF
        if b.numel() == 0:
            return scale.contiguous(), torch.zeros_like(scale)
        mi = torch.where(has_mean, mean_idx, torch.zeros_like(mean_idx))
        shift = torch.where(has_mean, b[mi] - rm[mi] * scale, torch.zeros_like(scale))
        return scale.contiguous(), shift.contiguous()

    def forward(self, data: DataKey.Type) -> DataKey.Type:
        x = data[DataKey.NODE_FEATURES]
        fuse = None
        if not _ag.needs_grad_lazy(lambda: (x, *_geometry(data), *_ag.params_of(self.conv), *_ag.params_of(self.norm))) \
                and x.shape[0] >= AGG_KM_MIN_ROWS:
            fuse = self._gate_fuse_args(x.device)
        self.conv.__dict__["_gate_fuse"] = fuse
        try:
            data = self.conv(data)
        finally:
            self.conv.__dict__["_gate_fuse"] = None
        if data.pop(GATE_APPLIED, False):
            return data
        data[DataKey.NODE_FEATURES] = self.act(data[DataKey.NODE_FEATURES], self.norm, data)
        return data
```

### matten_amd/nn/utils.py

```python
import os
from typing import Callable, Dict, List, Optional

import numpy as np
import torch
from torch import Tensor

from .. import autograd as _ag
from .. import ops, plan as _plan
from ..data.irreps import DataKey, ModuleIrreps
from ..o3 import Irrep, Irreps
from ._activation import act_const_table, normalize2mom_const
from ._tables import DerivedWeight, DeviceTables

ACTIVATION = {"e": {"ssp": "ssp", "silu": "silu", "sigmoid": "sigmoid"}, "o": {"abs": "abs", "tanh": "tanh"}}

tp_path_exists = _plan.tp_path_exists


def _inverse_permutation(gather):
    import numpy as np

    g = np.asarray(gather).reshape(-1)
    assert g.size == 0 or (np.sort(g) == np.arange(g.size)).all(), "packed weight table is not a permutation"
    inv = np.empty_like(g)
# ... 155 lines not shown
        w0p[:nb] = w0 / nb**0.5
        w1p = self._pack_mid(ws[:-1])
        w2p = ws[-1].new_zeros(h, w_pad)
        w2p[:, :W] = ws[-1] * (self.act_cst / h**0.5)
        return w0p, w1p, w2p

    def forward_train(self, geom_sorted: Tensor, n_basis: int, r_start: float, r_end: float) -> Tensor:
        if n_basis != self.hs[0]:
            raise ValueError(f"radial basis size {n_basis} != MLP input {self.hs[0]}")
        return _ag.RadialMLPFn.apply(self, geom_sorted, n_basis, r_start, r_end, *self.weights())

    def _hidden_one(self, geom_sorted: Tensor, n_basis: int, r_start: float, r_end: float, w0p, w1p) -> Tensor:
        fn = ops.radial_hidden_deep if self.deep else ops.radial_hidden
        return fn(geom_sorted, n_basis, r_start, r_end, w0p, w1p, self.h_scale(r_start, r_end))

    def hidden(self, geom_sorted: Tensor, n_basis: int, r_start: float, r_end: float, data=None):
        if n_basis != self.hs[0]:
            raise ValueError(f"radial basis size {n_basis} != MLP input {self.hs[0]}")
        w0p, w1p, w2p = self._packed.get(*self.weights())
        src = self.__dict__.get("_hidden_from")
        if src is not None:
            return src.hidden(geom_sorted, n_basis, r_start, r_end, data)[0], w2p
        group = radial_group_of(self)
        if data is not None and len(group) > 1 and os.environ.get("MATTEN_RADIAL_MULTI", "1") != "0" and \
                all(m.hs[:-1] == self.hs[:-1] for m in group):
            cache = data.get("_amd_h2s")
            if cache is None or cache.get("geom") is not geom_sorted or id(self) not in cache:
                packs = [m._packed.get(*m.weights()) for m in group]
                fn = ops.radial_hidden_multi_deep if self.deep else ops.radial_hidden_multi
                outs = fn(geom_sorted, n_basis, r_start, r_end, [p[0] for p in packs], [p[1] for p in packs],
                          [m.h_scale(r_start, r_end) for m in group])
                cache = {"geom": geom_sorted, **{id(m): h for m, h in zip(group, outs)}}
                data["_amd_h2s"] = cache
            return cache.pop(id(self)), w2p
        return self._hidden_one(geom_sorted, n_basis, r_start, r_end, w0p, w1p), w2p


_HUB_SPLIT_LEN_ENV = os.environ.get("MATTEN_HUB_SPLIT_LEN")
HUB_SPLIT_LEN = int(_HUB_SPLIT_LEN_ENV) if _HUB_SPLIT_LEN_ENV is not None else 16


def hub_split_len(n_rows: int) -> int:
    if _HUB_SPLIT_LEN_ENV is not None:
        return HUB_SPLIT_LEN
    return 8 if n_rows <= 768 else (16 if n_rows <= 3072 else 32)


HUB_SPLIT_MAX_ROWS = int(os.environ.get("MATTEN_HUB_SPLIT_MAX_ROWS", "8192"))
TRAIN_FUSED_MIN_EDGES = int(os.environ.get("MATTEN_TRAIN_TP_FUSED_MIN_EDGES", "65536"))


class UVUTensorProduct(torch.nn.Module):
    def __init__(
        self,
        irreps_in1: Irreps,
        irreps_in2: Irreps,
        irreps_out: Irreps,
        *,
        internal_and_share_weights: bool = False,
        mlp_input_size: int = None,
        mlp_hidden_size: int = 8,
        mlp_num_hidden_layers: int = 1,
        mlp_activation: str = "ssp",
    ):
        super().__init__()
        if internal_and_share_weights:
            raise NotImplementedError("internal shared weights are not used by the model factories")
        assert mlp_input_size is not None, (
            "Expect `mlp_input_size` be provided when `internal_and_share_weights` is set to `False`, got `None`"
        )
        self.plan = _plan.plan_uvu(irreps_in1, irreps_in2, irreps_out)
        self.irreps_mid = self.plan.irreps_mid
        self.weight_numel = self.plan.weight_numel
        layer_sizes = [mlp_input_size] + mlp_num_hidden_layers * [mlp_hidden_size] + [self.weight_numel]
        self.impl = os.environ.get("MATTEN_TP_IMPL", "fused")
        self._train_tp_auto = None
        if self.impl not in ("fused", "paths"):
            raise ValueError(f"MATTEN_TP_IMPL={self.impl!r}: 'fused' or 'paths' (the table-driven and block kernels of "
                             "rounds 1-2 were removed in round 4)")
        self.weight_nn = RadialMLP(layer_sizes, act=mlp_activation,
                                   out_cols=self.plan.fused_cols if self.impl == "fused" else None)
        self._tables = DeviceTables(
            entries=self.plan.path_entries, unit_start=self.plan.unit_start,
            gentries=self.plan.group_entries, gumap=self.plan.fused_unit_map,
            bw_col_meta=self.plan.bw_col_meta, bw_nnz_ijk=self.plan.bw_nnz_ijk, bw_nnz_c=self.plan.bw_nnz_c,
            bw_in_ptr=self.plan.bw_in_ptr, bw_in_cols=self.plan.bw_in_cols,
            bw_blocks=self.plan.bw_blocks, bw_paths=self.plan.bw_paths, bw_w_entries=self.plan.bw_w_entries,
            fused_cols=self.plan.fused_cols,
        )

        self._a_split = DerivedWeight(self._split_last_layer)
        self._a_split_c = None

    def _split_last_layer(self, *ws: Tensor):
        w2p = self.weight_nn._packed.get(*ws)[2]
        frag, scale_inv = ops.split_a_tiles(w2p, self.plan.group_entries)
        return frag, (scale_inv * self.weight_nn._h_scale.get(*ws[:-1])[1]).contiguous()

    def a_split(self, r_start: float, r_end: float):
        mlp = self.weight_nn
        mlp.h_scale(r_start, r_end)
        c = float(r_end - r_start)
        if c != self._a_split_c:
            self._a_split_c = c
            self._a_split._key = None
        return self._a_split.get(*mlp.weights())

    @property
    def irreps_out(self) -> Irreps:
        return self.irreps_mid.simplify()

    def forward(self, node_feats: Tensor, data: DataKey.Type, avg_num_neighbors=None, out_layout=None) -> Tensor:
        nb, r0, r1 = data[DataKey.AMD_RBF].tolist()
        dev = node_feats.device
        avg = avg_num_neighbors if avg_num_neighbors is not None else 0.0
        num_neigh = None if avg_num_neighbors is not None else data[DataKey.NUM_NEIGH]
        geom_grad = _ag.needs_grad(data[DataKey.AMD_GEOM], data[DataKey.AMD_SH])
        if geom_grad or _ag.needs_grad_lazy(lambda: (node_feats, *_ag.params_of(self.weight_nn))):
            from ._nequip import ensure_training_edge_tensors

            ensure_training_edge_tensors(data)
            mode = os.environ.get("MATTEN_TRAIN_TP", "auto")
            n_edges = data[DataKey.AMD_SRC].shape[0]
            if geom_grad:
                if os.environ.get("MATTEN_TP_BWD", "lit") != "lit":
                    raise NotImplementedError("MATTEN_TP_BWD=table has no adjoint for the edge harmonics: geometry "
                                              "gradients need MATTEN_TP_BWD=lit (the default)")
                mode = "paths"
            elif mode == "auto":
                if self._train_tp_auto is None:
                    self._train_tp_auto = "fused" if n_edges >= TRAIN_FUSED_MIN_EDGES else "paths"
                mode = self._train_tp_auto
            if self.impl == "fused" and mode == "fused":
                return _ag.FusedTensorProductFn.apply(node_feats, self, data, avg, num_neigh, *self.weight_nn.weights())
            w_edge = self.weight_nn.forward_train(data[DataKey.AMD_GEOM], int(nb), r0, r1)
            return _ag.TensorProductScatterFn.apply(node_feats, w_edge, data[DataKey.AMD_SH], self, data, avg, num_neigh)
        if self.impl == "fused":
            h2p, w2p = self.weight_nn.hidden(data[DataKey.AMD_GEOM], int(nb), r0, r1, data)
            rowptr = data[DataKey.AMD_ROWPTR]
            split = None
            piece = hub_split_len(node_feats.shape[0])
            if out_layout is None and piece > 0 and node_feats.shape[0] < HUB_SPLIT_MAX_ROWS:
                key = ("_amd_csr_split", piece, num_neigh is None)
                split = data.get(key)
                if split is None or split[3] is not rowptr:
                    split = ops.csr_split(rowptr, data[DataKey.AMD_SRC].shape[0], piece, num_neigh) + (rowptr,)
                    data[key] = split
            agg = ops.tp_fused(
                node_feats, h2p, w2p, data[DataKey.AMD_SH], rowptr if split is None else split[0], data[DataKey.AMD_SRC],
                out_layout[0] if out_layout is not None else self._tables.get("gentries", dev),
                self._tables.get("gumap", dev), len(self.plan.fused_unit_map),
                self.plan.fused_lds_floats_per_wave, out_layout[1] if out_layout is not None else self.plan.d_mid, avg,
                num_neigh if split is None else split[2], a_split=self.a_split(r0, r1),
            )
            return agg if split is None else ops.segment_reduce(agg, split[1], mean=False)
        w_edge = self.weight_nn(data[DataKey.AMD_GEOM], int(nb), r0, r1)
        return ops.tp_paths(
            node_feats, w_edge, data[DataKey.AMD_SH], data[DataKey.AMD_ROWPTR], data[DataKey.AMD_SRC],
            self._tables.get("entries", dev), self._tables.get("unit_start", dev), self.plan.units_per_tile,
            self.plan.d_mid, avg, num_neigh,
        )


def _n_valid(data):
    return data.get(DataKey.AMD_N_VALID) if data is not None else None


class ActivationLayer(torch.nn.Module):
    def __init__(
        self,
        tp_irreps_in1: Irreps,
        tp_irreps_in2: Irreps,
        tp_irreps_out: Irreps,
        *,
        activation_type: str = "gate",
        activation_scalars: Dict[str, str] = None,
        activation_gates: Dict[str, str] = None,
    ):
        super().__init__()
        key = {"e": 1, "o": -1}
        scal = {1: "ssp", -1: "tanh"} if activation_scalars is None else {
            key[k]: ACTIVATION[k][v] for k, v in activation_scalars.items()
        }
        gat = {1: "ssp", -1: "abs"} if activation_gates is None else {
            key[k]: ACTIVATION[k][v] for k, v in activation_gates.items()
        }
        self.activation_type = activation_type
        if activation_type == "norm":
            self.plan = _plan.plan_norm_act(tp_irreps_in1, tp_irreps_in2, tp_irreps_out, scal)
            self._tables = DeviceTables(chan=self.plan.chan)
            return
        if activation_type != "gate":
            supported = ("gate", "norm")
            raise ValueError(f"Support `activation_type` includes {supported}, got {activation_type}")
        self.plan = _plan.plan_gate(tp_irreps_in1, tp_irreps_in2, tp_irreps_out, scal, gat)
        self._tables = DeviceTables(meta=self.plan.meta, act_cst=act_const_table().numpy())

    @property
    def irreps_in(self) -> Irreps:
        return self.plan.irreps_in

    @property
    def irreps_out(self) -> Irreps:
        return self.plan.irreps_out

    def _forward_norm_act(self, x: Tensor, norm, data) -> Tensor:
        dev = x.device
        bn = norm.n if (norm is not None and norm.method == "batch") else None
        if bn is not None and not bn.training and _ag.needs_grad(x, bn.weight, bn.bias):
            return _ag.NormActBnEvalFn.apply(x, bn.weight, bn.bias, self, bn)
        if _ag.needs_grad(x) or (bn is not None and bn.training) or (norm is not None and norm.method == "instance"):
            y = _ag.NormActFn.apply(x, self) if _ag.needs_grad(x) else ops.norm_act(
                x, self._tables.get("chan", dev), self.plan.act_code, self.plan.epsilon)
            if norm is not None and norm.method == "instance":
                return norm.n(y, data)
            if bn is None:
                return y
            return bn.forward_train(y, _n_valid(data))
        return ops.norm_act(x, self._tables.get("chan", dev), self.plan.act_code, self.plan.epsilon,
                            *((bn.running_mean, bn.running_var, bn.weight, bn.bias, bn.eps) if bn is not None else ()))

    def forward(self, x: Tensor, norm: "NormalizationLayer" = None, data=None) -> Tensor:
        dev = x.device
        if self.activation_type == "norm":
            return self._forward_norm_act(x, norm, data)
        if norm is not None and norm.method == "instance":
            y = _ag.GateFn.apply(x, self) if _ag.needs_grad(x) else ops.gate_bn(
                x, self._tables.get("meta", dev), self._tables.get("act_cst", dev))
            return norm.n(y, data)
        bn = norm.n if (norm is not None and norm.n is not None) else None
        if bn is not None and bn.training:
            y = _ag.GateFn.apply(x, self) if x.requires_grad else ops.gate_bn(
                x, self._tables.get("meta", dev), self._tables.get("act_cst", dev))
            return bn.forward_train(y, _n_valid(data))
        if bn is not None and _ag.needs_grad(x, bn.weight, bn.bias):
            return _ag.GateBnEvalFn.apply(x, bn.weight, bn.bias, self, bn)
        if _ag.needs_grad(x):
            return _ag.GateFn.apply(x, self)
        return ops.gate_bn(
            x, self._tables.get("meta", dev), self._tables.get("act_cst", dev),
            *((bn.running_mean, bn.running_var, bn.weight, bn.bias) if bn is not None else (None, None, None, None)),
            eps=bn.eps if bn is not None else 1e-5,
        )


class _IrrepBatchNorm(torch.nn.Module):

    def __init__(self, irreps: Irreps, eps: float = 1e-5, momentum: float = 0.1):
        super().__init__()
        self.irreps = Irreps(irreps)
        self.eps, self.momentum = eps, momentum
        n_scalar = sum(m for m, ir in self.irreps if ir.is_scalar())
        n_feat = self.irreps.num_irreps
        self.register_buffer("running_mean", torch.zeros(n_scalar))
        self.register_buffer("running_var", torch.ones(n_feat))
        self.weight = torch.nn.Parameter(torch.ones(n_feat))
        self.bias = torch.nn.Parameter(torch.zeros(n_scalar))
        chan, col2chan = _plan.plan_batchnorm(self.irreps)
        self._tables = DeviceTables(chan=chan, col2chan=col2chan,
                                    scalar_chan=np.nonzero(chan[:, 2])[0].astype(np.int64))

    def forward_train(self, x: Tensor, n_valid: Tensor = None) -> Tensor:
        if n_valid is None:
            return _ag.BatchNormTrainFn.apply(x, self.weight, self.bias, self)
        return _ag.BatchNormTrainFn.apply(x, self.weight, self.bias, self, n_valid)

    def train(self, mode: bool = True):
        return super().train(mode and not self.__dict__.get("_frozen_stats", False))


class _IrrepInstanceNorm(torch.nn.Module):

    def __init__(self, irreps: Irreps, eps: float = 1e-5):
        super().__init__()
        self.irreps = Irreps(irreps)
        self.eps = eps
        n_scalar = sum(m for m, ir in self.irreps if ir.l == 0)
        self.weight = torch.nn.Parameter(torch.ones(self.irreps.num_irreps))
        self.bias = torch.nn.Parameter(torch.zeros(n_scalar))
        chan, col2chan = _plan.plan_batchnorm(self.irreps, odd_scalars_too=True)
        self._tables = DeviceTables(chan=chan, col2chan=col2chan,
                                    scalar_chan=np.nonzero(chan[:, 2])[0].astype(np.int64))

    def forward(self, x: Tensor, data) -> Tensor:
        from ._nequip import with_batch

        with_batch(data)
        batch = data[DataKey.BATCH]
        ptr = data.get(DataKey.PTR)
        if ptr is None:
            n_seg = int(batch[-1]) + 1 if batch.numel() else 1
            ptr = torch.searchsorted(batch, torch.arange(n_seg + 1, device=batch.device, dtype=batch.dtype))
        if _ag.needs_grad(x, self.weight, self.bias):
            return _ag.InstanceNormFn.apply(x, self.weight, self.bias, self, ptr, batch)
        dev = x.device
        return ops.instance_norm_fwd(x, ptr, batch, self._tables.get("col2chan", dev), self._tables.get("chan", dev),
                                     self.weight, self.bias, self.eps)[0]


class NormalizationLayer(torch.nn.Module):
    def __init__(self, irreps: Irreps, method: str = None):
        super().__init__()
        self.method = method
        supported = ("batch", "instance", "none", None)
        assert method in supported, f"Unsupported normalization {method}"
        self.n = _IrrepBatchNorm(irreps) if method == "batch" else _IrrepInstanceNorm(irreps) if method == "instance" else None
# ... 21 lines not shown
```

### matten_amd/ops.py

```python
from __future__ import annotations

from typing import Optional, Tuple

import os

import numpy as np

import torch

from . import _lib
from .nn._tables import bump_weights_epoch


_EVENTS = None
_EVENTS_ONLY = None


def enable_event_timing(flag: bool = True, only=None) -> None:
    global _EVENTS, _EVENTS_ONLY
    _EVENTS = {} if flag else None
    _EVENTS_ONLY = tuple(only) if (flag and only) else None


def event_timings_ms():
# ... 392 lines not shown
    with _timed(f"radial_mlp_bwd/w_pad={w_pad}"):
        rc = lib.matten_radial_mlp_bwd(_ptr(geom_sorted), E, n_basis, r_start, r_end, _ptr(w0p), nb_pad, _ptr(w1p),
                                       _ptr(w2p), hidden, w_pad, int(w_cols), _ptr(dw), dw.shape[1],
                                       int(dw.dtype == torch.bfloat16), _ptr(h2), _ptr(part_small), _ptr(part_w2),
                                       float(scales[0]), float(scales[1]), float(scales[2]), _ptr(small), _ptr(d2),
                                       _stream())
    _lib.check(rc, "matten_radial_mlp_bwd")
    return small[: nb_pad * hidden].reshape(nb_pad, hidden), small[nb_pad * hidden:].reshape(hidden, hidden), d2


def tp_paths(x, w_edge, sh_sorted, rowptr, src_sorted, entries, unit_start, units_per_tile: int, d_mid: int,
             avg_num_neighbors: float, num_neigh=None) -> torch.Tensor:
    lib = _lib.load()
    from .plan import TP_TILE_NODES

    if lib.matten_tp_tile_nodes() != TP_TILE_NODES:
        raise _lib.MattenHipError("plan.TP_TILE_NODES does not match the library's node tile")
    x = _need(x, torch.float32, "node_features")
    w_edge = _edge_dtype(w_edge, "w_edge")
    sh_sorted = _need(sh_sorted, torch.float32, "sh_sorted")
    N, d_in = rowptr.shape[0] - 1, x.shape[1]
    if num_neigh is not None:
        num_neigh = _need(num_neigh, torch.float32, "num_neigh")
    agg = torch.empty(N, d_mid, dtype=torch.float32, device=x.device)
    with _timed(f"tp_scatter/d_mid={d_mid}"):
        rc = lib.matten_tp_paths(_ptr(x), d_in, _ptr(w_edge), w_edge.shape[1], _ptr(sh_sorted), sh_sorted.shape[1],
                                 _ptr(rowptr), _ptr(src_sorted), N, _ptr(entries), _ptr(unit_start),
                                 entries.shape[0], units_per_tile, d_mid, float(avg_num_neighbors or 0.0),
                                 _ptr(num_neigh), _ptr(agg), int(w_edge.dtype == torch.bfloat16), _stream())
    _lib.check(rc, "matten_tp_paths")
    return agg


def split_hidden(h2p: torch.Tensor) -> torch.Tensor:
    tiny = 2.0 ** -14
    hi = torch.where(h2p.abs() < tiny, torch.zeros_like(h2p), h2p.half().float())
    lo = (h2p - hi) * 2048.0
    lo = torch.where(lo.abs() < tiny, torch.zeros_like(lo), lo)
    return torch.stack([hi.half(), lo.half()], dim=1).contiguous()


def radial_hidden(geom_sorted, n_basis: int, r_start: float, r_end: float, w0p, w1p, h_scale=None) -> torch.Tensor:
    lib = _lib.load()
    geom_sorted = _need(geom_sorted, torch.float32, "geom_sorted")
    w0p, w1p = _need(w0p, torch.float32, "w0p"), _need(w1p, torch.float32, "w1p")
    E = geom_sorted.shape[0]
    h2p = torch.empty(E, 2, 32, dtype=torch.float16, device=geom_sorted.device)
    with _timed("radial_hidden"):
        if h_scale is not None:
            h_scale = _need(h_scale, torch.float32, "h_scale")
        rc = lib.matten_radial_hidden(_ptr(geom_sorted), E, n_basis, r_start, r_end, _ptr(w0p), w0p.shape[0],
                                      _ptr(w1p), w0p.shape[1], _ptr(h2p), _ptr(h_scale), _stream())
    _lib.check(rc, "matten_radial_hidden")
    return h2p


def radial_hidden_multi(geom_sorted, n_basis: int, r_start: float, r_end: float, w0ps, w1ps, h_scales=None):
    import ctypes

    lib = _lib.load()
    geom_sorted = _need(geom_sorted, torch.float32, "geom_sorted")
    w0ps = [_need(w, torch.float32, "w0p") for w in w0ps]
    w1ps = [_need(w, torch.float32, "w1p") for w in w1ps]
    L, E = len(w0ps), geom_sorted.shape[0]
    if not 1 <= L <= 8 or len(w1ps) != L or any(w.shape != w0ps[0].shape for w in w0ps):
        raise ValueError("radial_hidden_multi: 1..8 layers with equal basis / hidden sizes")
    out = [torch.empty(E, 2, 32, dtype=torch.float16, device=geom_sorted.device) for _ in range(L)]
    arr = lambda ts: (ctypes.c_void_p * L)(*[t.data_ptr() for t in ts])
    if h_scales is not None:
        h_scales = [_need(h, torch.float32, "h_scale") for h in h_scales]
        if len(h_scales) != L:
            raise ValueError("one h_scale per layer")
    with _timed("radial_hidden_multi"):
        rc = lib.matten_radial_hidden_multi(_ptr(geom_sorted), E, n_basis, r_start, r_end, arr(w0ps), w0ps[0].shape[0],
                                            arr(w1ps), w0ps[0].shape[1], arr(out),
                                            arr(h_scales) if h_scales is not None else None, L, _stream())
    _lib.check(rc, "matten_radial_hidden_multi")
    return out


def radial_hidden_deep(geom_sorted, n_basis: int, r_start: float, r_end: float, w0p, w_mid, h_scale=None) -> torch.Tensor:
    lib = _lib.load()
    geom_sorted = _need(geom_sorted, torch.float32, "geom_sorted")
    w0p = _need(w0p, torch.float32, "w0p")
    w_mid, n_mid = _mid(w_mid, "w_mid")
    E = geom_sorted.shape[0]
    h2p = torch.empty(E, 2, 32, dtype=torch.float16, device=geom_sorted.device)
    with _timed("radial_hidden"):
        if h_scale is not None:
            h_scale = _need(h_scale, torch.float32, "h_scale")
        rc = lib.matten_radial_hidden_deep(_ptr(geom_sorted), E, n_basis, r_start, r_end, _ptr(w0p), w0p.shape[0],
                                           _ptr(w_mid), n_mid, w0p.shape[1], _ptr(h2p), _ptr(h_scale), _stream())
    _lib.check(rc, "matten_radial_hidden_deep")
    return h2p


def radial_hidden_multi_deep(geom_sorted, n_basis: int, r_start: float, r_end: float, w0ps, w_mids, h_scales=None):
    import ctypes

    lib = _lib.load()
    geom_sorted = _need(geom_sorted, torch.float32, "geom_sorted")
    w0ps = [_need(w, torch.float32, "w0p") for w in w0ps]
    mids = [_mid(w, "w_mid") for w in w_mids]
    L, E = len(w0ps), geom_sorted.shape[0]
    if not 1 <= L <= 8 or len(mids) != L or any(w.shape != w0ps[0].shape for w in w0ps) or \
            any(m[1] != mids[0][1] for m in mids):
        raise ValueError("radial_hidden_multi_deep: 1..8 layers with equal basis / hidden sizes and depth")
    n_mid = mids[0][1]
    out = [torch.empty(E, 2, 32, dtype=torch.float16, device=geom_sorted.device) for _ in range(L)]
    arr = lambda ts: (ctypes.c_void_p * L)(*[t.data_ptr() for t in ts])
    if h_scales is not None:
        h_scales = [_need(h, torch.float32, "h_scale") for h in h_scales]
        if len(h_scales) != L:
            raise ValueError("one h_scale per layer")
    with _timed("radial_hidden_multi"):
        rc = lib.matten_radial_hidden_multi_deep(_ptr(geom_sorted), E, n_basis, r_start, r_end, arr(w0ps), w0ps[0].shape[0],
                                                 arr([m[0] for m in mids]) if n_mid else None, n_mid, w0ps[0].shape[1],
                                                 arr(out), arr(h_scales) if h_scales is not None else None, L, _stream())
    _lib.check(rc, "matten_radial_hidden_multi_deep")
    return out


def split_a_tiles(w2p: torch.Tensor, group_entries) -> Tuple[torch.Tensor, torch.Tensor]:
    dev = w2p.device
    g = torch.arange(4, device=dev)[:, None]
    kk = torch.arange(8, device=dev)[None, :]
    k_idx = 16 * (kk >> 2) + 4 * g + (kk & 3)
    tiny = 2.0 ** -14
    tiles, inv = [], []
    for row in np.asarray(group_entries).reshape(-1, 32):
        w_base, n_mt = int(row[5]), int(row[7])
        if int(row[0]) < 0 or n_mt == 0:
            inv.append(torch.ones((), device=dev))
            continue
        A = w2p[k_idx][:, :, w_base:w_base + 16 * n_mt]
        A = A.reshape(4, 8, n_mt, 16).permute(2, 0, 3, 1)
        amax = A.abs().max()
        e = torch.where(amax > 0, (torch.frexp(amax)[1] - 1).clamp(-100, 100), torch.full_like(amax, 13, dtype=torch.int32))
        scale = torch.ldexp(torch.ones_like(amax), 13 - e)
        inv.append(torch.ldexp(torch.ones_like(amax), e - 13))
        v = A * scale
        hi = torch.where(v.abs() < tiny, torch.zeros_like(v), v.half().float())
        lo = (v - hi) * 2048.0
        lo = torch.where(lo.abs() < tiny, torch.zeros_like(lo), lo)
        tiles.append(torch.cat([hi.half(), lo.half()], dim=-1).reshape(n_mt, 64, 16))
    return torch.cat(tiles).contiguous(), torch.stack(inv).float().contiguous()


_GROUPS_CHECKED = False


def tp_fused(x, h2p, w2p, sh_sorted, rowptr, src_sorted, entries, unit_map, units_per_tile: int,
             lds_floats_per_wave: int, d_mid: int, avg_num_neighbors: float, num_neigh=None,
             a_split=None) -> torch.Tensor:
    lib = _lib.load()
    from .plan import TP_TILE_NODES

    if lib.matten_tp_tile_nodes() != TP_TILE_NODES:
        raise _lib.MattenHipError("plan.TP_TILE_NODES does not match the library's node tile")
    from .plan import TP_MAX_COLS, TP_MAX_COLS_L0, TP_MAX_COLS_L1
    if (lib.matten_tp_max_cols() != TP_MAX_COLS or lib.matten_tp_max_cols_l0() != TP_MAX_COLS_L0
            or lib.matten_tp_max_cols_l1() != TP_MAX_COLS_L1):
        raise _lib.MattenHipError("plan.TP_MAX_COLS does not match the library's entry width (-DTPF_MAX_COLS)")
    from .plan import TP_WREG_MAX_L1, tp_wreg
    if tp_wreg() and lib.matten_tp_wreg() != TP_WREG_MAX_L1 + 1:
        raise _lib.MattenHipError("plans mark coupling-major entries (plan.TP_KIND_WREG) that this library was not built for "
                                  "(-DTPF_WREG=0 / -DTPF_WREG_MAX_L1): set MATTEN_TP_WREG=0")
    global _GROUPS_CHECKED
    from .plan import tp_groups_hash
    if not _GROUPS_CHECKED and lib.matten_tp_groups_hash() != tp_groups_hash():
        raise _lib.MattenHipError("the library's coupling code (cg_gen.h) was generated for other coupling groups than plan.TP_GROUPS "
                                  "(MATTEN_TP_GROUPS / an interrupted tools/*.sh A/B build?): make -C matten_amd/csrc clean all")
    _GROUPS_CHECKED = True
    x = _need_rows(x, torch.float32, "node_features")
    h2p = _need(h2p, torch.float16, "h2s")
    if h2p.dim() != 3 or h2p.shape[1:] != (2, 32):
        raise ValueError(f"h2s must be [E,2,32] fp16 (ops.split_hidden / ops.radial_hidden), got {tuple(h2p.shape)}")
    w2p = _need(w2p, torch.float32, "w2p")
    sh_sorted = _need(sh_sorted, torch.float32, "sh_sorted")
    N, d_in = rowptr.shape[0] - 1, x.stride(0)
    if num_neigh is not None:
        num_neigh = _need(num_neigh, torch.float32, "num_neigh")
    if a_split is not None:
        a_split = (_need(a_split[0], torch.float16, "a_split"), _need(a_split[1], torch.float32, "a_scale_inv"))
        if a_split[1].numel() != entries.shape[0]:
            raise ValueError("a_scale_inv needs one value per group entry")
    if unit_map.numel() != units_per_tile:
        raise ValueError(f"unit_map has {unit_map.numel()} units, expected {units_per_tile} (plan.fused_unit_map)")
    agg = torch.empty(N, d_mid, dtype=torch.float32, device=x.device)
    with _timed(f"tp_scatter/d_mid={d_mid}/d_in={x.shape[1]}"):
        rc = lib.matten_tp_fused(_ptr(x), d_in, _ptr(h2p), _ptr(w2p), w2p.shape[1], _ptr(sh_sorted),
                                 sh_sorted.shape[1], _ptr(rowptr), _ptr(src_sorted), N, _ptr(entries),
                                 _ptr(unit_map), entries.shape[0], units_per_tile, lds_floats_per_wave, d_mid,
                                 float(avg_num_neighbors or 0.0), _ptr(num_neigh),
                                 _ptr(a_split[0]) if a_split is not None else None,
                                 _ptr(a_split[1]) if a_split is not None else None, _ptr(agg), _stream())
    _lib.check(rc, "matten_tp_fused")
    return agg


def agg_linear(agg, species_order, wtab, io_table, blocks, d_out: int, add=None) -> torch.Tensor:
    lib = _lib.load()
    from .plan import AGG_BLOCK, AGG_MAX_MT
    if lib.matten_agg_linear_block_chunks() != AGG_BLOCK or lib.matten_agg_linear_max_mt() != AGG_MAX_MT:
        raise _lib.MattenHipError("plan.AGG_BLOCK / AGG_MAX_MT do not match the library (-DAL_BLK_CHUNKS)")
    agg = _need(agg, torch.float32, "agg")
    wtab = _need(wtab, torch.float32, "A fragments")
    n_rows, ld = agg.shape
    order, seg = species_order if species_order is not None else (None, None)
    n_species = wtab.shape[0] if wtab.dim() == 2 else 1
    if add is not None:
        add = _need_rows(add, torch.float32, "add")
    out = torch.empty(n_rows, d_out, dtype=torch.float32, device=agg.device)
    with _timed(f"agg_linear/ld={ld}"):
        rc = lib.matten_agg_linear(_ptr(agg), ld, _ptr(order), _ptr(seg), n_species, _ptr(wtab), wtab.shape[-1],
                                   _ptr(io_table), io_table.shape[0], _ptr(blocks), blocks.shape[0], _ptr(add),
                                   add.stride(0) if add is not None else d_out, d_out, n_rows, _ptr(out), _stream())
    _lib.check(rc, "matten_agg_linear")
    return out


def agg_linear_gate(agg, species_order, wtab, io_table, blocks, d_out: int, cmeta, act_cst, d_act: int, add=None,
                    bn_scale=None, bn_shift=None) -> torch.Tensor:
    lib = _lib.load()
    from .plan import AGG_BLOCK, AGG_GATE_SETS, AGG_MAX_MT
    if (lib.matten_agg_linear_block_chunks() != AGG_BLOCK or lib.matten_agg_linear_max_mt() != AGG_MAX_MT
            or lib.matten_agg_linear_gate_sets() != AGG_GATE_SETS):
        raise _lib.MattenHipError("plan.AGG_BLOCK / AGG_MAX_MT / AGG_GATE_SETS do not match the library")
    agg = _need(agg, torch.float32, "agg")
    wtab = _need(wtab, torch.float32, "A fragments")
    n_rows, ld = agg.shape
    order, seg = species_order if species_order is not None else (None, None)
    n_species = wtab.shape[0] if wtab.dim() == 2 else 1
    if add is not None:
        add = _need_rows(add, torch.float32, "add")
    if cmeta.shape != (d_out, 4):
        raise ValueError("cmeta must be [d_out, 4]")
    if bn_scale is not None:
        bn_scale, bn_shift = _need(bn_scale, torch.float32, "bn_scale"), _need(bn_shift, torch.float32, "bn_shift")
        if bn_scale.numel() != d_act or bn_shift.numel() != d_act:
            raise ValueError("bn_scale / bn_shift must have one value per activated column")
    out = torch.empty(n_rows, d_act, dtype=torch.float32, device=agg.device)
    with _timed(f"agg_linear/ld={ld}"):
        rc = lib.matten_agg_linear_gate(_ptr(agg), ld, _ptr(order), _ptr(seg), n_species, _ptr(wtab), wtab.shape[-1],
                                        _ptr(io_table), io_table.shape[0], _ptr(blocks), blocks.shape[0], _ptr(add),
                                        add.stride(0) if add is not None else d_out, d_out, n_rows, _ptr(cmeta),
                                        _ptr(act_cst), _ptr(bn_scale), _ptr(bn_shift), d_act, _ptr(out), _stream())
    _lib.check(rc, "matten_agg_linear_gate")
    return out


_SL_ROWS_LDS_BYTES = 52 * 1024


def species_linear_route(d_in: int, w_stride: int, n_items_per_pass) -> str:
    n_items = list(n_items_per_pass)
    fits = len(n_items) == 1 and 4 * (16 * (d_in | 1) + w_stride + 8 * n_items[0] + 4) <= _SL_ROWS_LDS_BYTES
    return "rows" if fits else "stream"


def species_linear(x, species_order, wp, w_stride: int, item_tables, d_out: int, add=None,
                   fully_covered: bool = True, variant: Optional[str] = None) -> torch.Tensor:
    lib = _lib.load()
    x = _need(x, torch.float32, "x")
    from . import selfcheck
    selfcheck.check_species_linear(x.device)
    wp = _need(wp, torch.float32, "packed weights")
    n_rows, d_in = x.shape
    order, seg = species_order if species_order is not None else (None, None)
    n_species = wp.shape[0] if wp.dim() == 2 else 1
    cur_add = add
    if cur_add is not None:
        cur_add = _need_rows(cur_add, torch.float32, "add")
    if fully_covered:
        out = torch.empty(n_rows, d_out, dtype=torch.float32, device=x.device)
    else:
        out = cur_add.clone() if cur_add is not None else torch.zeros(n_rows, d_out, dtype=torch.float32, device=x.device)
    rows_fits = species_linear_route(d_in, w_stride, [t.shape[0] for t in item_tables]) == "rows"
    rows_variant = rows_fits and os.environ.get("MATTEN_SL_ROWS", "1") != "0"
    if variant is not None:
        rows_variant = rows_fits and variant == "rows"
    for items in item_tables:
        fn = lib.matten_species_linear_rows if rows_variant else lib.matten_species_linear
        _lib.check(
            fn(_ptr(x), d_in, _ptr(order), _ptr(seg), n_species, _ptr(wp), w_stride,
                                      _ptr(items), items.shape[0], d_out, _ptr(cur_add),
                                      cur_add.stride(0) if cur_add is not None else d_out, n_rows, _ptr(out), _stream()),
            "matten_species_linear",
        )
        cur_add = out
    return out


def gate_bn(x, meta, act_cst, running_mean=None, running_var=None, bn_weight=None, bn_bias=None, eps: float = 1e-5):
    lib = _lib.load()
    x = _need(x, torch.float32, "x")
    n_rows, d_in = x.shape
    d_out = meta.shape[0]
    out = torch.empty(n_rows, d_out, dtype=torch.float32, device=x.device)
    _lib.check(
        lib.matten_gate_bn(_ptr(x), d_in, _ptr(meta), d_out, _ptr(act_cst), _ptr(running_mean), _ptr(running_var),
                           _ptr(bn_weight), _ptr(bn_bias), eps, n_rows, _ptr(out), _stream()),
        "matten_gate_bn",
    )
    return out


def segment_reduce(x, ptr, mean: bool) -> torch.Tensor:
    lib = _lib.load()
    x = _need(x, torch.float32, "x")
    ptr = _need(ptr, torch.int64, "ptr")
    B = ptr.shape[0] - 1
    out = torch.empty(B, x.shape[1], dtype=torch.float32, device=x.device)
    _lib.check(lib.matten_segment_reduce(_ptr(x), x.shape[1], _ptr(ptr), B, int(mean), _ptr(out), _stream()),
               "matten_segment_reduce")
    return out


def segment_minmax(x, ptr, take_max: bool, want_arg: bool = False):
    lib = _lib.load()
    x = _need(x, torch.float32, "x")
    ptr = _need(ptr, torch.int64, "ptr")
    B = ptr.shape[0] - 1
    out = torch.empty(B, x.shape[1], dtype=torch.float32, device=x.device)
    arg = torch.empty(B, x.shape[1], dtype=torch.int64, device=x.device) if want_arg else None
    _lib.check(lib.matten_segment_minmax(_ptr(x), x.shape[1], _ptr(ptr), B, int(take_max), _ptr(out), _ptr(arg), _stream()),
               "matten_segment_minmax")
    return (out, arg) if want_arg else out


def segment_minmax_bwd(dy, arg, n_rows: int) -> torch.Tensor:
    lib = _lib.load()
    dy = _need(dy, torch.float32, "dy")
    dx = torch.zeros(n_rows, dy.shape[1], dtype=torch.float32, device=dy.device)
    _lib.check(lib.matten_segment_minmax_bwd(_ptr(dy), dy.shape[1], _ptr(arg), dy.shape[0], _ptr(dx), _stream()),
               "matten_segment_minmax_bwd")
    return dx


def dense_rows(x, q) -> torch.Tensor:
    lib = _lib.load()
    x = _need(x, torch.float32, "x")
# ... 1138 lines not shown
```

### matten_amd/plan.py

```python
from __future__ import annotations

import math
import os
from dataclasses import dataclass, field
from typing import Dict, List, Optional, Sequence, Tuple

import numpy as np

from .o3 import Irrep, Irreps, wigner_3j

TP_TILE_NODES = 64

def _range_groups(ranges, l1, lmax=4):
    return [[(l2, l3) for l2 in range(lo, hi + 1) for l3 in range(abs(l1 - l2), min(lmax, l1 + l2) + 1)] for lo, hi in ranges]


def _moved(l1, to_first, lmax=4):
    g0, g1 = _range_groups([(0, 2), (3, 4)], l1, lmax)
    assert all(c in g1 for c in to_first)
    return [g0 + list(to_first), [c for c in g1 if c not in to_first]]


_GROUP_SCHEMES = {
    "A": {l1: _range_groups([(0, 4)] if l1 == 0 else [(0, 2), (3, 4)], l1) for l1 in range(5)},
# ... 611 lines not shown
        (ii, io)
        for ii, (_, iri) in enumerate(irreps_in)
        for io, (_, iro) in enumerate(irreps_out)
        if iri == iro
    ]
    return _plan_linear_like(irreps_in, irreps_out, 1, paths)


@dataclass
class GatePlan:
    irreps_in: Irreps
    irreps_out: Irreps
    irreps_scalars: Irreps
    irreps_gates: Irreps
    irreps_gated: Irreps
    meta: np.ndarray
    n_bn_features: int
    n_bn_scalars: int


def plan_gate(tp_irreps_in1, tp_irreps_in2, tp_irreps_out, act_scalars: Dict[int, str],
              act_gates: Dict[int, str]) -> GatePlan:
    tp_irreps_out = Irreps(tp_irreps_out).sort()[0].simplify()
    scalars = Irreps(
        [(m, ir) for m, ir in tp_irreps_out if ir.l == 0 and tp_path_exists(tp_irreps_in1, tp_irreps_in2, ir)]
    )
    gated = Irreps(
        [(m, ir) for m, ir in tp_irreps_out if ir.l > 0 and tp_path_exists(tp_irreps_in1, tp_irreps_in2, ir)]
    )
    if gated.dim > 0:
        if tp_path_exists(tp_irreps_in1, tp_irreps_in2, "0e"):
            gir = Irrep("0e")
        elif tp_path_exists(tp_irreps_in1, tp_irreps_in2, "0o"):
            gir = Irrep("0o")
        else:
            raise ValueError(
                f"tp_irreps_in1={tp_irreps_in1} times tp_irreps_in2={tp_irreps_in2} is unable to produce gates "
                f"needed for irreps_gated={gated}"
            )
        gates = Irreps([(m, gir) for m, _ in gated]).simplify()
    else:
        gates = Irreps([])
    scalars, gates, gated = scalars.simplify(), gates.simplify(), gated.simplify()

    cat = scalars + gates + gated
    sorted_ir, p, _ = cat.sort()
    offs = sorted_ir.offsets()
    pos = [offs[p[i]] for i in range(len(cat))]
    ns, ng = len(scalars), len(gates)
    irreps_in = sorted_ir.simplify()

    rows: List[Tuple[int, int, int, int]] = []
    out_ir: List[Tuple[int, Irrep]] = []
    bn_idx = 0
    mean_idx = 0
    for b, (m, ir) in enumerate(scalars):
        name = act_scalars[ir.p]
        ir_o = Irrep(0, _scalar_out_parity(name, ir.p))
        for u in range(m):
            mi = (mean_idx + u) if ir_o.is_scalar() else 0xFFFF
            rows.append((pos[b] + u, -1, ACT_CODE[name], (bn_idx + u) | (mi << 16)))
        if ir_o.is_scalar():
            mean_idx += m
        bn_idx += m
        out_ir.append((m, ir_o))
    gate_chan: List[Tuple[int, int]] = []
    for b, (m, ir) in enumerate(gates):
        gate_chan += [(pos[ns + b] + u, ir.p) for u in range(m)]
    gc = 0
    for b, (m, ir) in enumerate(gated):
        d = ir.dim
        p_gate = 1
        for u in range(m):
            gpos, gp = gate_chan[gc]
            gc += 1
            gname = act_gates[gp]
            p_gate = _scalar_out_parity(gname, gp)
            for k in range(d):
                rows.append((pos[ns + ng + b] + u * d + k, gpos, ACT_CODE[gname] << 8, (bn_idx + u) | (0xFFFF << 16)))
        bn_idx += m
        out_ir.append((m, Irrep(ir.l, ir.p * p_gate)))
    irreps_out = Irreps(out_ir)
    meta = np.array(rows, dtype=np.int64).reshape(-1, 4)
    meta = np.where(meta >= 2**31, meta - 2**32, meta).astype(np.int32)
    assert meta.shape[0] == irreps_out.dim
    return GatePlan(irreps_in, irreps_out, scalars, gates, gated, meta, irreps_out.num_irreps,
                    sum(m for m, ir in irreps_out if ir.is_scalar()))


@dataclass
class NormActPlan:
    irreps_in: Irreps
    irreps_out: Irreps
    chan: np.ndarray
    act_code: int
    epsilon: float = 1e-8


def plan_norm_act(tp_irreps_in1, tp_irreps_in2, tp_irreps_out, act_scalars: Dict[int, str]) -> NormActPlan:
    tp_irreps_out = Irreps(tp_irreps_out).sort()[0].simplify()
    scalars = Irreps([(m, ir) for m, ir in tp_irreps_out if ir.l == 0 and tp_path_exists(tp_irreps_in1, tp_irreps_in2, ir)])
    gated = Irreps([(m, ir) for m, ir in tp_irreps_out if ir.l > 0 and tp_path_exists(tp_irreps_in1, tp_irreps_in2, ir)])
    irreps = (scalars + gated).simplify()
    chan, _ = plan_batchnorm(irreps)
    return NormActPlan(irreps, irreps, chan, ACT_CODE[act_scalars[1]])


_ACT_PARITY = {"silu": 0, "ssp": 0, "sigmoid": 0, "tanh": -1, "abs": 1}


def _scalar_out_parity(act_name: str, p_in: int) -> int:
    if p_in == 1:
        return 1
    pa = _ACT_PARITY[act_name]
    if pa == 0:
        raise ValueError(f"activation {act_name} on an odd scalar violates parity")
    return pa


def plan_batchnorm(irreps, odd_scalars_too: bool = False) -> Tuple[np.ndarray, np.ndarray]:
    irreps = Irreps(irreps)
    chan, col2chan = [], []
    off = 0
    mi = 0
    for mul, ir in irreps:
        for _ in range(mul):
            is0 = 1 if (ir.l == 0 if odd_scalars_too else ir.is_scalar()) else 0
            chan.append((off, ir.dim, is0, mi if is0 else -1))
            col2chan += [len(chan) - 1] * ir.dim
            off += ir.dim
            mi += is0
    return np.array(chan, dtype=np.int32).reshape(-1, 4), np.array(col2chan, dtype=np.int32)


AGG_CHUNK = 16
AGG_BLOCK = int(os.environ.get("MATTEN_AGG_BLOCK", "4"))
AGG_STAGE_W = 32
AGG_ROW_CUT = os.environ.get("MATTEN_AGG_ROW_CUT", "component")
AGG_MAX_MT = 2


@dataclass
class AggLinearPlan:
    entries: np.ndarray
    ld: int
    n_chunks: int
    io_table: np.ndarray
    blocks: np.ndarray
    w_stride: int
    gather: np.ndarray
    scale: np.ndarray
    d_out: int
    max_mt: int


AGG_GATE_SETS = 3


def _bw_wfree_lds(bw_blocks, cap: int = 4096) -> int:
    need = 2048
    for _x, mul, _l, w in bw_blocks:
        cu = 1 << max(0, (int(mul) - 1).bit_length())
        need = max(need, (256 // cu) * ((int(w) >> 16) * ((int(mul) + 3) // 4 * 4) + 4))
    return int(min(cap, -(-need // 64) * 64))


def plan_agg_gate(ap: "AggLinearPlan", gate: "GatePlan") -> Optional[np.ndarray]:
    meta = np.asarray(gate.meta).reshape(-1, 4)
    d_conv = int(ap.d_out)
    rows = [(int(r[5]), int(r[6]), int(r[3] & 255), int(r[7]), int((r[3] >> 24) & 255))
            for r in np.asarray(ap.io_table).reshape(-1, 8)]

    def row_of(col):
        for ii, (o, mo, d3, k0, kk) in enumerate(rows):
            if o <= col < o + mo * d3 and k0 <= (col - o) % d3 < k0 + kk:
                return ii, (col - o) // d3 * kk + (col - o) % d3 - k0
        return None

    cm = np.zeros((d_conv, 4), dtype=np.int64)
    gate_cols = {}
    for o, (src, gcol, codes, _bn) in enumerate(meta):
        act, gact = int(codes) & 255, (int(codes) >> 8) & 255
        if gcol < 0:
            cm[src] = (1 | (act << 8), o, 0, 0)
        else:
            gate_cols.setdefault(int(gcol), gact)
            cm[src] = (3, o, int(gcol), -1)
    set_of_row = {}
    for gcol in sorted(gate_cols):
        where = row_of(gcol)
        if where is None:
            return None
        ii, lane = where
        st = set_of_row.setdefault(ii, len(set_of_row))
        if st >= AGG_GATE_SETS or lane >= 32:
            return None
        cm[gcol] = (2 | (gate_cols[gcol] << 8), 0, lane, st)
    first_user = {}
    for src in range(d_conv):
        if cm[src][0] & 255 == 3:
            gcol = int(cm[src][2])
            g_row = row_of(gcol)[0]
            u_row = row_of(src)
            if u_row is None or u_row[0] <= g_row:
                return None
            cm[src][2], cm[src][3] = cm[gcol][2], cm[gcol][3]
    if any((cm[c][0] & 255) == 0 for c in range(d_conv)):
        return None
    return cm.astype(np.int32)


def plan_agg_linear(uvu: UVUPlan, n_species: int, irreps_out) -> Optional[AggLinearPlan]:
    irreps_out = Irreps(irreps_out).simplify()
    S = n_species
    ent = np.asarray(uvu.group_entries).reshape(-1, 32).copy()
    mid = uvu.irreps_mid
    blk_of_slot, uoff_of_slot, blocks = [], [], []
    for mul, ir in mid:
        if blocks and blocks[-1][1] == ir:
            blk_of_slot.append(len(blocks) - 1)
            uoff_of_slot.append(blocks[-1][0])
            blocks[-1] = (blocks[-1][0] + mul, ir)
        else:
            blk_of_slot.append(len(blocks))
            uoff_of_slot.append(0)
            blocks.append((mul, ir))
    flat_of, fan, flat = {}, {}, 0
    for ib, (mi, ir) in enumerate(blocks):
        for io, (mo, iro) in enumerate(irreps_out):
            if iro == ir:
                flat_of[(ib, io)] = flat
                flat += mi * S * mo
                fan[io] = fan.get(io, 0) + mi * S
    o_offs = irreps_out.offsets()
    pieces: Dict[int, List[Tuple[int, int, int]]] = {}
    for e in range(len(ent)):
        for c, pi in sorted(uvu.group_entry_paths[e].items()):
            pth = uvu.paths[pi]
            ir3 = Irrep(pth.l3, pth.p3)
            ios = [io for io, (_, iro) in enumerate(irreps_out) if iro == ir3]
            if len(ios) != 1:
                return None
            pieces.setdefault(ios[0], []).append((e, c, int(uvu.group_entry_mul[e])))
    if any(io not in pieces for io in range(len(irreps_out)) if irreps_out[io].dim > 0):
        return None
    io_rows, gather_parts, scale_parts = [], [], []
    chunk0, a_off, max_mt = 0, 0, 1
    for io, (mo, iro) in enumerate(irreps_out):
        if iro.dim == 0 or mo == 0:
            continue
        d3 = iro.dim
        plist = sorted(pieces[io], key=lambda t: (-(1 << max(0, (t[2] - 1).bit_length())), t[0], t[1]))
        slot_src: List[Tuple[int, int]] = []
        piece_off = {}
        for (e, c, mul_c) in plist:
            width = 1 << max(0, (mul_c - 1).bit_length())
            while len(slot_src) % min(width, AGG_CHUNK):
                slot_src.append((-1, -1))
            piece_off[(e, c)] = len(slot_src)
            pth = uvu.paths[uvu.group_entry_paths[e][c]]
            ib = blk_of_slot[pth.slot]
            for uu in range(mul_c):
                slot_src.append((ib, uoff_of_slot[pth.slot] + uvu.group_entry_u0[e] + uu))
        if any(sb < 0 for sb, _ in slot_src):
            return None
        K = len(slot_src)
        T = -(-K // AGG_CHUNK)
        Kpad = T * AGG_CHUNK
        for (e, c, _) in plist:
            ent[e][8 + 12 + c] = chunk0 * AGG_CHUNK + piece_off[(e, c)]
            ent[e][8 + c] = Kpad
        step = 16 * AGG_MAX_MT
        while AGG_ROW_CUT == "channel" and step * d3 > AGG_STAGE_W and step > 1:
            step //= 2
        for v0 in range(0, mo, step):
            mo_p = min(step, mo - v0)
            n_mt = -(-mo_p // 16)
            cw = 16 if mo_p >= 16 else mo_p
            max_mt = max(max_mt, n_mt)
            t_, mt_, g_, c_, s_ = np.meshgrid(np.arange(T), np.arange(n_mt), np.arange(4), np.arange(cw), np.arange(4), indexing="ij")
            slot = (16 * t_ + 4 * g_ + s_).reshape(-1)
            v = (v0 + 16 * mt_ + c_).reshape(-1)
            src = np.array(slot_src + [(-1, -1)] * (Kpad - K), dtype=np.int64)
            ib_, u_ = src[slot, 0], src[slot, 1]
            base = np.array([flat_of.get((int(b), io), 0) for b in ib_], dtype=np.int64)
            g0 = base + u_ * S * mo + v
            valid = (ib_ >= 0) & (v < mo)
            gather_parts.append(np.where(valid[None, :], g0[None, :] + np.arange(S)[:, None] * mo, -1))
            scale_parts.append(np.full(slot.size, fan[io] ** -0.5, dtype=np.float32))
            kmax = max(1, AGG_STAGE_W // mo_p)
            for k0 in range(0, d3, kmax):
                kk = min(kmax, d3 - k0)
                io_rows.append((chunk0, T, K, d3 | (n_mt << 8) | (cw << 16) | (kk << 24), a_off, o_offs[io] + v0 * d3, mo_p, k0))
            a_off += slot.size
        chunk0 += d3 * T
    ld = -(-(chunk0 * AGG_CHUNK) // 32) * 32
    blocks = []
    for ii, (c0, T, K, packed, _a, _o, _m, k0) in enumerate(io_rows):
        kk = (packed >> 24) & 255
        for k in range(k0, k0 + kk):
            for t0 in range(0, T, AGG_BLOCK):
                n = min(AGG_BLOCK, T - t0)
                last = t0 + n == T
                blocks.append((c0 + k * T + t0, n | (int(t0 == 0) << 8) | (int(last) << 9)
                               | (int(last and k == k0 + kk - 1) << 10) | (k << 12) | (ii << 20), t0, 0))
    gather = np.concatenate(gather_parts, axis=1).astype(np.int64)
    assert gather.max() < flat
    return AggLinearPlan(entries=ent.astype(np.int32), ld=ld, n_chunks=chunk0,
                         io_table=np.array(io_rows, dtype=np.int32).reshape(-1, 8),
                         blocks=np.array(blocks, dtype=np.int32).reshape(-1, 4), w_stride=a_off, gather=gather,
                         scale=np.concatenate(scale_parts), d_out=irreps_out.dim, max_mt=max_mt)
```

Baseline: 1.288 billion edge-TP/s.

## Contract narrow-output TP paths with species weights in the scatter epilogue

For low-l, write-register tensor-product groups whose output multiplicity is smaller than the channel width, the epilogue now applies the per-species output linear weights directly, using DPP cross-lane reductions. It stores only the mo outputs per node instead of the full mul_c channels. The aggregation plan shrinks its leading dimension and puts identity weights in those slots. This cuts agg buffer width, store traffic and downstream linear work, at the cost of extra epilogue arithmetic, per-node species lookups and more complex weight packing. The narrow plan is used by default when it gives a smaller ld.

Result: faster. 1.321 billion edge-TP/s, median of 6 (+2.6%).

```diff
diff --git a/include/matten_hip.h b/include/matten_hip.h
--- a/include/matten_hip.h
+++ b/include/matten_hip.h
@@ -96,6 +96,13 @@
                     int64_t units_per_tile, int64_t lds_floats_per_wave, int64_t d_mid, float avg_num_neighbors,
                     const float* num_neigh, const uint16_t* a_split, const float* a_scale_inv,
                     float* agg , matten_stream_t stream);
+int matten_tp_fused_narrow(const float* x, int64_t d_in, const uint16_t* h2s, const float* w2p, int64_t w_pad,
+                           const float* sh_sorted, int64_t sh_stride, const int32_t* rowptr, const int32_t* src_sorted,
+                           int64_t n_nodes, const int32_t* group_entries, const int32_t* unit_map, int64_t n_entries,
+                           int64_t units_per_tile, int64_t lds_floats_per_wave, int64_t d_mid, float avg_num_neighbors,
+                           const float* num_neigh, const uint16_t* a_split, const float* a_scale_inv,
+                           const int32_t* species, float* agg , matten_stream_t stream);
+int matten_tp_narrow_max_l1(void);
 
 int matten_tp_wreg(void);
 int matten_tp_max_cols(void);
diff --git a/matten_amd/_lib.py b/matten_amd/_lib.py
--- a/matten_amd/_lib.py
+++ b/matten_amd/_lib.py
@@ -46,6 +46,8 @@
     "matten_tp_max_cols_l1": (c_int, []),
     "matten_tp_groups_hash": (c_int, []),
     "matten_tp_fused": (c_int, [P, c_int64, P, P, c_int64, P, c_int64, P, P, c_int64, P, P, c_int64, c_int64, c_int64, c_int64, c_float, P, P, P, P, P]),
+    "matten_tp_fused_narrow": (c_int, [P, c_int64, P, P, c_int64, P, c_int64, P, P, c_int64, P, P, c_int64, c_int64, c_int64, c_int64, c_float, P, P, P, P, P, P]),
+    "matten_tp_narrow_max_l1": (c_int, []),
     "matten_species_linear": (c_int, [P, c_int64, P, P, c_int64, P, c_int64, P, c_int64, c_int64, P, c_int64, c_int64, P, P]),
     "matten_species_linear_rows": (c_int, [P, c_int64, P, P, c_int64, P, c_int64, P, c_int64, c_int64, P, c_int64, c_int64, P, P]),
     "matten_radial_mlp_bwd_small_slices": (c_int64, [c_int64]),
diff --git a/matten_amd/csrc/tp_fused.hip b/matten_amd/csrc/tp_fused.hip
--- a/matten_amd/csrc/tp_fused.hip
+++ b/matten_amd/csrc/tp_fused.hip
@@ -6,10 +6,132 @@
 
 constexpr int KIND_MERGED = 256;
 constexpr int KIND_WREG = 512;
+constexpr int KIND_NARROW = 1024;
+#ifndef TPF_NARROW_MAX_L1
+#define TPF_NARROW_MAX_L1 1
+#endif
+
+#define TPF_DPP_ADD(d, s, CTRL, BANKS) \
+    asm volatile("s_nop 1\n\tv_add_f32_dpp %0, %1, %1 " CTRL " row_mask:0xf bank_mask:" BANKS : "+v"(d) : "v"(s))
+
+template <int CUL, int D3>
+__device__ __forceinline__ void narrow_sum(const float (&t)[D3], float* __restrict__ q) {
+    constexpr int NB = CUL == 4 ? 4 : 2;
+    constexpr int M = (D3 + NB - 1) / NB;
+    if constexpr (CUL == 4) {
+        float h[2 * M];
+#pragma unroll
+        for (int i = 0; i < 2 * M; ++i) {
+            const int k0 = (i >> 1) * 4 + (i & 1);
+            if (k0 < D3) {
+                h[i] = t[k0];
+                TPF_DPP_ADD(h[i], t[k0], "row_ror:8", "0x3");
+                if (k0 + 2 < D3) TPF_DPP_ADD(h[i], t[k0 + 2 < D3 ? k0 + 2 : 0], "row_ror:8", "0xc");
+            }
+        }
+#pragma unroll
+        for (int m = 0; m < M; ++m) {
+            q[m] = h[2 * m];
+            TPF_DPP_ADD(q[m], h[2 * m], "row_half_mirror", "0x5");
+            if (4 * m + 1 < D3) TPF_DPP_ADD(q[m], h[2 * m + 1], "row_half_mirror", "0xa");
+        }
+    } else {
+#pragma unroll
+        for (int m = 0; m < M; ++m) {
+            q[m] = t[2 * m];
+            TPF_DPP_ADD(q[m], t[2 * m], "row_half_mirror", "0x5");
+            if (2 * m + 1 < D3) TPF_DPP_ADD(q[m], t[2 * m + 1 < D3 ? 2 * m + 1 : 0], "row_half_mirror", "0xa");
+        }
+    }
+#pragma unroll
+    for (int m = 0; m < M; ++m) {
+        TPF_DPP_ADD(q[m], q[m], "quad_perm:[1,0,3,2]", "0xf");
+        TPF_DPP_ADD(q[m], q[m], "quad_perm:[2,3,0,1]", "0xf");
+    }
+}
+
+template <int CUL, int D3>
+__device__ __forceinline__ void narrow_coupling(const float* __restrict__ accp, const float* __restrict__ wp, int mo, float norm,
+                                                float* __restrict__ op, int ks, int u, bool valid) {
+    constexpr int NB = CUL == 4 ? 4 : 2;
+    constexpr int M = (D3 + NB - 1) / NB;
+    float w[4] = {0.0f, 0.0f, 0.0f, 0.0f};
+    if (mo == 4) {
+        const f32x4 v4 = *reinterpret_cast<const f32x4*>(wp);
+        w[0] = v4[0], w[1] = v4[1], w[2] = v4[2], w[3] = v4[3];
+    } else if (mo == 2) {
+        const float2 v2 = *reinterpret_cast<const float2*>(wp);
+        w[0] = v2.x, w[1] = v2.y;
+    } else {
+        w[0] = wp[0];
+    }
+    float q[4][M];
+#pragma unroll
+    for (int v = 0; v < 4; ++v) {
+#pragma unroll
+        for (int m = 0; m < M; ++m) q[v][m] = 0.0f;
+        if (v < mo) {
+            const float wv = w[v] * norm;
+            float t[D3];
+#pragma unroll
+            for (int k = 0; k < D3; ++k) t[k] = accp[k] * wv;
+            narrow_sum<CUL, D3>(t, q[v]);
+        }
+    }
+    const int l = u & 3, b = (u >> 2) & (NB - 1);
+#pragma unroll
+    for (int m = 0; m < M; ++m) {
+        const int k = b + NB * m;
+        if (valid && l == (m & 3) && k < D3) {
+            float* p = op + k * ks;
+            if (mo == 4) {
+                const f32x4 r = {q[0][m], q[1][m], q[2][m], q[3][m]};
+                *reinterpret_cast<f32x4*>(p) = r;
+            } else if (mo == 2) {
+                *reinterpret_cast<float2*>(p) = make_float2(q[0][m], q[1][m]);
+            } else {
+                *p = q[0][m];
+            }
+        }
+    }
+}
+
 struct StoreAgg {
-    template <class G>
-    __device__ __forceinline__ void store(const Args& a, const GroupEntry& ge, const float* __restrict__ acc,
+    template <class G, int CULH>
+    __device__ __forceinline__ unsigned store_narrow(const Args& a, const GroupEntry& ge, const float* __restrict__ acc,
+                                                     float a_scale_inv, int node, int u, bool valid) const {
+        const int nsafe = min(node, a.n_nodes - 1);
+        const float nn = a.avg_nn > 0.0f ? a.avg_nn : a.num_neigh[nsafe];
+        const float norm = nn > 0.0f ? a_scale_inv / sqrtf(nn) : 0.0f;
+        const int sp = a.species[nsafe];
+        float* orow = a.agg + (int64_t)node * a.d_mid;
+        const int cul = CULH ? CULH : ge.cu_log2;
+        unsigned done = 0;
+        for_slots<0, G::NC, 1>([&](auto cc_) {
+            constexpr int cc = decltype(cc_)::value;
+            constexpr int D3 = 2 * G::L3[cc] + 1;
+            const unsigned tw = (unsigned)ge.t_off[cc];
+            const int mo = (int)(tw >> 20);
+            if (mo != 0) {
+                done |= 1u << cc;
+                const unsigned ow = (unsigned)ge.out_off[cc];
+                const float* wp = reinterpret_cast<const float*>(&ge) + 4 * (int)(ow >> 16) + ((sp << cul) + u) * mo;
+                float* op = orow + (int)(ow & 0xffffu);
+                const int ks = (int)(tw & 0xfffffu);
+                if (cul == 4) narrow_coupling<4, D3>(acc + G::OFF[cc], wp, mo, norm, op, ks, u, valid);
+                else narrow_coupling<3, D3>(acc + G::OFF[cc], wp, mo, norm, op, ks, u, valid);
+            }
+        });
+        return done;
+    }
+
+    template <class G, int CULH>
+    __device__ __forceinline__ void store(const Args& a, const GroupEntry& ge, const float* acc,
                                           float a_scale_inv, int node, int j, int u, bool valid) const {
+        unsigned narrowed = 0;
+        if constexpr (CULH >= 0 && G::D1 <= 2 * TPF_NARROW_MAX_L1 + 1 && !TPF_LAB_NO_STORE) {
+            if (a.species && (ge.kind & KIND_NARROW)) narrowed = store_narrow<G, CULH>(a, ge, acc, a_scale_inv, node, u, valid);
+        }
         if (TPF_LAB_NO_STORE ? (valid && acc[0] == 12345.678f) : valid) {
             const float nn = a.avg_nn > 0.0f ? a.avg_nn : a.num_neigh[node];
             const float norm = nn > 0.0f ? a_scale_inv / sqrtf(nn) : 0.0f;
@@ -17,7 +139,7 @@
             const bool merged = (ge.kind & KIND_MERGED) != 0;
             const GroupEntry& g2 = (&ge)[merged ? 1 : 0];
             const bool second = merged && u >= 2;
-            const unsigned mask = merged ? (second ? g2.mask : (unsigned)g2.w_base) : ge.mask;
+            const unsigned mask = (merged ? (second ? g2.mask : (unsigned)g2.w_base) : ge.mask) & ~narrowed;
             const int uc = second ? u - 2 : u;
 #pragma unroll
             for (int cc = 0; cc < G::NC; ++cc) {
@@ -166,7 +288,7 @@
         }
         __builtin_amdgcn_wave_barrier();
     }
-    StoreAgg{}.store<G>(a, ge, acc, a_scale_inv, node, j, u, valid);
+    StoreAgg{}.store<G, 0>(a, ge, acc, a_scale_inv, node, j, u, valid);
 }
 
 #define MATTEN_RGS_ARGS a, ge, tile, stage, (um >> 8) & 0xffff, tile_id, r, reps, lane, StoreAgg{}
@@ -597,13 +719,13 @@
 }
 #endif
 
-extern "C" int matten_tp_fused(const float* x, int64_t d_in, const uint16_t* h2s, const float* w2p, int64_t w_pad,
-                               const float* sh_sorted, int64_t sh_stride, const int32_t* rowptr,
-                               const int32_t* src_sorted, int64_t n_nodes, const int32_t* group_entries,
-                               const int32_t* unit_map, int64_t n_entries, int64_t units_per_tile,
-                               int64_t lds_floats_per_wave, int64_t d_mid, float avg_num_neighbors,
-                               const float* num_neigh, const uint16_t* a_split, const float* a_scale_inv, float* agg,
-                               matten_stream_t stream_) {
+static int tp_fused_launch(const float* x, int64_t d_in, const uint16_t* h2s, const float* w2p, int64_t w_pad,
+                           const float* sh_sorted, int64_t sh_stride, const int32_t* rowptr,
+                           const int32_t* src_sorted, int64_t n_nodes, const int32_t* group_entries,
+                           const int32_t* unit_map, int64_t n_entries, int64_t units_per_tile,
+                           int64_t lds_floats_per_wave, int64_t d_mid, float avg_num_neighbors,
+                           const float* num_neigh, const uint16_t* a_split, const float* a_scale_inv,
+                           const int32_t* species, float* agg, matten_stream_t stream_) {
     hipStream_t stream = (hipStream_t)stream_;
     if (n_nodes < 0 || d_in <= 0 || w_pad <= 0 || sh_stride < 32 || (sh_stride & 3) || n_entries <= 0 ||
         units_per_tile <= 0 || d_mid <= 0 || lds_floats_per_wave <= 0 || (lds_floats_per_wave & 3))
@@ -616,7 +738,8 @@
     if (lds > 64 * 1024) return MATTEN_EINVAL;
     if ((a_split == nullptr) != (a_scale_inv == nullptr)) return MATTEN_EINVAL;
     Args a{x, (const _Float16*)h2s, w2p, (const _Float16*)a_split, a_scale_inv, sh_sorted, rowptr, src_sorted, num_neigh, agg, (int)d_in, (int)w_pad, (int)sh_stride,
-           (int)d_mid, (int)n_nodes, (int)lds_floats_per_wave, avg_num_neighbors};
+           (int)d_mid, (int)n_nodes, (int)lds_floats_per_wave, avg_num_neighbors,
+           species};
     const int n_tiles = (int)matten_cdiv(n_nodes, TILE_NODES);
     const int blocks_per_tile = (int)matten_cdiv(units_per_tile, WAVES_PER_BLOCK);
     const int64_t grid = matten_cdiv(n_tiles, N_XCD) * N_XCD * (int64_t)blocks_per_tile;
@@ -635,6 +758,32 @@
     return MATTEN_OK;
 }
 
+extern "C" int matten_tp_fused(const float* x, int64_t d_in, const uint16_t* h2s, const float* w2p, int64_t w_pad,
+                               const float* sh_sorted, int64_t sh_stride, const int32_t* rowptr,
+                               const int32_t* src_sorted, int64_t n_nodes, const int32_t* group_entries,
+                               const int32_t* unit_map, int64_t n_entries, int64_t units_per_tile,
+                               int64_t lds_floats_per_wave, int64_t d_mid, float avg_num_neighbors,
+                               const float* num_neigh, const uint16_t* a_split, const float* a_scale_inv, float* agg,
+                               matten_stream_t stream_) {
+    return tp_fused_launch(x, d_in, h2s, w2p, w_pad, sh_sorted, sh_stride, rowptr, src_sorted, n_nodes, group_entries, unit_map,
+                           n_entries, units_per_tile, lds_floats_per_wave, d_mid, avg_num_neighbors, num_neigh, a_split,
+                           a_scale_inv, nullptr, agg, stream_);
+}
+
+extern "C" int matten_tp_fused_narrow(const float* x, int64_t d_in, const uint16_t* h2s, const float* w2p, int64_t w_pad,
+                                      const float* sh_sorted, int64_t sh_stride, const int32_t* rowptr,
+                                      const int32_t* src_sorted, int64_t n_nodes, const int32_t* group_entries,
+                                      const int32_t* unit_map, int64_t n_entries, int64_t units_per_tile,
+                                      int64_t lds_floats_per_wave, int64_t d_mid, float avg_num_neighbors,
+                                      const float* num_neigh, const uint16_t* a_split, const float* a_scale_inv,
+                                      const int32_t* species, float* agg, matten_stream_t stream_) {
+    if (n_nodes > 0 && (!species || (d_mid & 3))) return MATTEN_EINVAL;
+    return tp_fused_launch(x, d_in, h2s, w2p, w_pad, sh_sorted, sh_stride, rowptr, src_sorted, n_nodes, group_entries, unit_map,
+                           n_entries, units_per_tile, lds_floats_per_wave, d_mid, avg_num_neighbors, num_neigh, a_split,
+                           a_scale_inv, species, agg, stream_);
+}
+
+extern "C" int matten_tp_narrow_max_l1(void) { return TPF_NARROW_MAX_L1; }
 extern "C" int matten_tp_wreg(void) { return TPF_WREG ? TPF_WREG_MAX_L1 + 1 : 0; }
 extern "C" int matten_tp_max_cols(void) { return TPF_MAX_COLS; }
 extern "C" int matten_tp_max_cols_l0(void) { return TPF_MAX_COLS_L0; }
diff --git a/matten_amd/csrc/tp_walk.h b/matten_amd/csrc/tp_walk.h
--- a/matten_amd/csrc/tp_walk.h
+++ b/matten_amd/csrc/tp_walk.h
@@ -171,6 +171,7 @@
     float* agg;
     int d_in, w_pad, sh_stride, d_mid, n_nodes, lds_per_wave;
     float avg_nn;
+    const int* species;
 #if TPF_TRACING
     unsigned* trace;
 #endif
@@ -834,7 +835,7 @@
 #if TPF_TRACING
     tr_epi_sg += (unsigned)(tpf_stamp() - tr_end);
 #endif
-    epi.template store<G>(a, ge, acc, a_scale_inv, node_done, j, u, valid_done);
+    epi.template store<G, (WR ? WR : -1)>(a, ge, acc, a_scale_inv, node_done, j, u, valid_done);
     if (!TPF_REP_PREFETCH && more) start_group(unit_nodes_finish(raw_next));
 #if TPF_TRACING
     if (a.trace && lane == 0) {
diff --git a/matten_amd/nn/conv.py b/matten_amd/nn/conv.py
--- a/matten_amd/nn/conv.py
+++ b/matten_amd/nn/conv.py
@@ -6,6 +6,7 @@
 
 from .. import autograd as _ag
 from .. import ops
+from .. import plan as _plan_mod
 from ..data.irreps import DataKey, ModuleIrreps
 from ..o3 import Irreps
 from ._tables import DerivedWeight, DeviceTables, WeightSlice
@@ -65,10 +66,17 @@
         self.agg_plan = None
         if self.tp.impl == "fused" and os.environ.get("MATTEN_AGG_LAYOUT", "km") == "km":
             ap = _plan.plan_agg_linear(self.tp.plan, n_species, conv_layer_irreps)
+            if ap is not None and os.environ.get("MATTEN_AGG_NARROW", "1") != "0":
+                apn = _plan.plan_agg_narrow(self.tp.plan, n_species, conv_layer_irreps)
+                if apn is not None and apn.ld < ap.ld and self._agg_fits(apn):
+                    ap = apn
             if ap is not None and self._agg_fits(ap):
                 self.agg_plan = ap
-                self._agg_tables = DeviceTables(entries=ap.entries, io=ap.io_table, blocks=ap.blocks, gather=ap.gather,
-                                                scale=ap.scale)
+                tables = dict(entries=ap.entries, io=ap.io_table, blocks=ap.blocks, gather=ap.gather, scale=ap.scale)
+                if ap.narrow is not None:
+                    tables.update(narrow_gather=ap.narrow_gather, narrow_scale=ap.narrow_scale)
+                    self._agg_narrow_w = DerivedWeight(self._pack_narrow_weights)
+                self._agg_tables = DeviceTables(**tables)
                 self._agg_wtab = DerivedWeight(self._pack_agg_weights)
 
     def _pack_lin1_sc(self, w1: torch.Tensor, w2: torch.Tensor) -> torch.Tensor:
@@ -100,7 +108,22 @@
     def _pack_agg_weights(self, w: torch.Tensor) -> torch.Tensor:
         t, dev = self._agg_tables, w.device
         gather, scale = t.get("gather", dev), t.get("scale", dev)
-        return torch.where(gather >= 0, w[gather.clamp(min=0)] * scale[None, :], w.new_zeros(())).contiguous()
+        one = (gather == _plan_mod.AGG_GATHER_ONE).to(w.dtype)
+        return torch.where(gather >= 0, w[gather.clamp(min=0)] * scale[None, :], one).contiguous()
+
+    def _pack_narrow_weights(self, w: torch.Tensor) -> torch.Tensor:
+        t, dev = self._agg_tables, w.device
+        wn = (w[t.get("narrow_gather", dev)] * t.get("narrow_scale", dev)).to(torch.float32).contiguous()
+        return torch.cat([t.get("entries", dev).reshape(-1), wn.view(torch.int32)])
+
+    def _agg_out_layout(self, data, dev):
+        ap, t = self.agg_plan, self._agg_tables
+        if ap.narrow is None:
+            return (t.get("entries", dev), ap.ld)
+        species = data.get(DataKey.AMD_SPECIES_I32)
+        if species is None:
+            raise ValueError("narrowed neighbour sums need the per-node species index (DataKey.AMD_SPECIES_I32)")
+        return (self._agg_narrow_w.get(self.lin2.weight), ap.ld, (species, len(ap.entries)))
 
     def build_inference_view(self, kept_irreps) -> bool:
         kept = Irreps(kept_irreps).simplify()
@@ -177,7 +200,7 @@
                 and not _ag.needs_grad_lazy(lambda: (x1, self_connection, self.lin2.weight, *_geometry(data),
                                                      *_ag.params_of(self.tp.weight_nn)))):
             ap, t, dev = self.agg_plan, self._agg_tables, x1.device
-            agg = self.tp(x1, data, self.avg_num_neighbors, out_layout=(t.get("entries", dev), ap.ld))
+            agg = self.tp(x1, data, self.avg_num_neighbors, out_layout=self._agg_out_layout(data, dev))
             gate = self.__dict__.get("_gate_fuse")
             if gate is not None:
                 cmeta, act_cst, d_act, bn_scale, bn_shift = gate
diff --git a/matten_amd/nn/utils.py b/matten_amd/nn/utils.py
--- a/matten_amd/nn/utils.py
+++ b/matten_amd/nn/utils.py
@@ -331,6 +331,7 @@
                 self._tables.get("gumap", dev), len(self.plan.fused_unit_map),
                 self.plan.fused_lds_floats_per_wave, out_layout[1] if out_layout is not None else self.plan.d_mid, avg,
                 num_neigh if split is None else split[2], a_split=self.a_split(r0, r1),
+                narrow=out_layout[2] if out_layout is not None and len(out_layout) > 2 else None,
             )
             return agg if split is None else ops.segment_reduce(agg, split[1], mean=False)
         w_edge = self.weight_nn(data[DataKey.AMD_GEOM], int(nb), r0, r1)
diff --git a/matten_amd/ops.py b/matten_amd/ops.py
--- a/matten_amd/ops.py
+++ b/matten_amd/ops.py
@@ -568,7 +568,7 @@
 
 def tp_fused(x, h2p, w2p, sh_sorted, rowptr, src_sorted, entries, unit_map, units_per_tile: int,
              lds_floats_per_wave: int, d_mid: int, avg_num_neighbors: float, num_neigh=None,
-             a_split=None) -> torch.Tensor:
+             a_split=None, narrow=None) -> torch.Tensor:
     lib = _lib.load()
     from .plan import TP_TILE_NODES
 
@@ -595,15 +595,33 @@
     w2p = _need(w2p, torch.float32, "w2p")
     sh_sorted = _need(sh_sorted, torch.float32, "sh_sorted")
     N, d_in = rowptr.shape[0] - 1, x.stride(0)
+    n_entries = entries.shape[0] if narrow is None else int(narrow[1])
     if num_neigh is not None:
         num_neigh = _need(num_neigh, torch.float32, "num_neigh")
     if a_split is not None:
         a_split = (_need(a_split[0], torch.float16, "a_split"), _need(a_split[1], torch.float32, "a_scale_inv"))
-        if a_split[1].numel() != entries.shape[0]:
+        if a_split[1].numel() != n_entries:
             raise ValueError("a_scale_inv needs one value per group entry")
     if unit_map.numel() != units_per_tile:
         raise ValueError(f"unit_map has {unit_map.numel()} units, expected {units_per_tile} (plan.fused_unit_map)")
     agg = torch.empty(N, d_mid, dtype=torch.float32, device=x.device)
+    if narrow is not None:
+        from .plan import AGG_NARROW_MAX_L1
+        if lib.matten_tp_narrow_max_l1() != AGG_NARROW_MAX_L1:
+            raise _lib.MattenHipError("plan.AGG_NARROW_MAX_L1 does not match the library (-DTPF_NARROW_MAX_L1)")
+        sp = _need(narrow[0], torch.int32, "species")
+        if sp.numel() != N or d_mid % 4 or entries.dim() != 1 or entries.numel() <= n_entries * 32:
+            raise ValueError("narrow: one species index per destination row, d_mid a multiple of 4, and `entries` the buffer of "
+                             "plan.narrow_blob (entries | weights)")
+        with _timed(f"tp_scatter/d_mid={d_mid}/d_in={x.shape[1]}"):
+            rc = lib.matten_tp_fused_narrow(_ptr(x), d_in, _ptr(h2p), _ptr(w2p), w2p.shape[1], _ptr(sh_sorted),
+                                            sh_sorted.shape[1], _ptr(rowptr), _ptr(src_sorted), N, _ptr(entries),
+                                            _ptr(unit_map), n_entries, units_per_tile, lds_floats_per_wave, d_mid,
+                                            float(avg_num_neighbors or 0.0), _ptr(num_neigh),
+                                            _ptr(a_split[0]) if a_split is not None else None,
+                                            _ptr(a_split[1]) if a_split is not None else None, _ptr(sp), _ptr(agg), _stream())
+        _lib.check(rc, "matten_tp_fused_narrow")
+        return agg
     with _timed(f"tp_scatter/d_mid={d_mid}/d_in={x.shape[1]}"):
         rc = lib.matten_tp_fused(_ptr(x), d_in, _ptr(h2p), _ptr(w2p), w2p.shape[1], _ptr(sh_sorted),
                                  sh_sorted.shape[1], _ptr(rowptr), _ptr(src_sorted), N, _ptr(entries),
diff --git a/matten_amd/plan.py b/matten_amd/plan.py
--- a/matten_amd/plan.py
+++ b/matten_amd/plan.py
@@ -787,6 +787,9 @@
     scale: np.ndarray
     d_out: int
     max_mt: int
+    narrow: Optional[np.ndarray] = None
+    narrow_gather: Optional[np.ndarray] = None
+    narrow_scale: Optional[np.ndarray] = None
 
 
 AGG_GATE_SETS = 3
@@ -846,6 +849,41 @@
 
 
 def plan_agg_linear(uvu: UVUPlan, n_species: int, irreps_out) -> Optional[AggLinearPlan]:
+    return _plan_agg(uvu, n_species, irreps_out, narrow=False)
+
+
+TP_KIND_NARROW = 1024
+AGG_NARROW_MAX_L1 = 1
+AGG_NARROW_MULS = (8, 16)
+AGG_NARROW_MO = (1, 2, 4)
+AGG_GATHER_ONE = -2
+
+
+def plan_agg_narrow(uvu: UVUPlan, n_species: int, irreps_out) -> Optional[AggLinearPlan]:
+    ap = _plan_agg(uvu, n_species, irreps_out, narrow=True)
+    return ap if ap is not None and ap.narrow is not None and ap.narrow.any() else None
+
+
+def narrow_blob(ap: AggLinearPlan, weights: np.ndarray) -> np.ndarray:
+    w = np.ascontiguousarray(weights, dtype=np.float32)
+    assert w.shape == ap.narrow_gather.shape
+    return np.concatenate([ap.entries.reshape(-1).astype(np.int32), w.view(np.int32)])
+
+
+def narrow_unpack(t_off_word: int, out_off_word: int):
+    t, o = int(t_off_word) & 0xFFFFFFFF, int(out_off_word) & 0xFFFFFFFF
+    mo = t >> 20
+    return (t & 0xFFFFF, o & 0xFFFF, mo, 4 * (o >> 16)) if mo else (t, o, 0, 0)
+
+
+def _narrows(ent_row, mul_c: int, mo: int) -> bool:
+    kind = int(ent_row[0])
+    return ((kind & 255) // TP_KIND_STRIDE <= AGG_NARROW_MAX_L1 and not kind & TP_KIND_MERGED and bool(kind & TP_KIND_WREG)
+            and mul_c in AGG_NARROW_MULS and (1 << int(ent_row[3])) == mul_c and int(ent_row[2]) == mul_c
+            and mo < mul_c and mo in AGG_NARROW_MO)
+
+
+def _plan_agg(uvu: UVUPlan, n_species: int, irreps_out, narrow: bool) -> Optional[AggLinearPlan]:
     irreps_out = Irreps(irreps_out).simplify()
     S = n_species
     ent = np.asarray(uvu.group_entries).reshape(-1, 32).copy()
@@ -869,6 +907,7 @@
                 fan[io] = fan.get(io, 0) + mi * S
     o_offs = irreps_out.offsets()
     pieces: Dict[int, List[Tuple[int, int, int]]] = {}
+    narrowed: Dict[Tuple[int, int], int] = {}
     for e in range(len(ent)):
         for c, pi in sorted(uvu.group_entry_paths[e].items()):
             pth = uvu.paths[pi]
@@ -876,10 +915,18 @@
             ios = [io for io, (_, iro) in enumerate(irreps_out) if iro == ir3]
             if len(ios) != 1:
                 return None
-            pieces.setdefault(ios[0], []).append((e, c, int(uvu.group_entry_mul[e])))
+            mul_c = int(uvu.group_entry_mul[e])
+            mo_c = int(irreps_out[ios[0]].mul)
+            if narrow and _narrows(ent[e], mul_c, mo_c):
+                narrowed[(e, c)] = mo_c
+                mul_c = mo_c
+            pieces.setdefault(ios[0], []).append((e, c, mul_c))
     if any(io not in pieces for io in range(len(irreps_out)) if irreps_out[io].dim > 0):
         return None
     io_rows, gather_parts, scale_parts = [], [], []
+    narrow_woff: Dict[Tuple[int, int], int] = {}
+    narrow_gather: List[np.ndarray] = []
+    narrow_scale: List[np.ndarray] = []
     chunk0, a_off, max_mt = 0, 0, 1
     for io, (mo, iro) in enumerate(irreps_out):
         if iro.dim == 0 or mo == 0:
@@ -895,9 +942,17 @@
             piece_off[(e, c)] = len(slot_src)
             pth = uvu.paths[uvu.group_entry_paths[e][c]]
             ib = blk_of_slot[pth.slot]
+            if (e, c) in narrowed:
+                slot_src.extend((AGG_GATHER_ONE, v) for v in range(mul_c))
+                mul_e, u_first = int(uvu.group_entry_mul[e]), uoff_of_slot[pth.slot] + uvu.group_entry_u0[e]
+                s_, u_, v_ = np.meshgrid(np.arange(S), np.arange(mul_e), np.arange(mo), indexing="ij")
+                narrow_woff[(e, c)] = sum(g.size for g in narrow_gather)
+                narrow_gather.append((flat_of[(ib, io)] + (u_first + u_) * S * mo + s_ * mo + v_).reshape(-1))
+                narrow_scale.append(np.full(narrow_gather[-1].size, fan[io] ** -0.5, dtype=np.float32))
+                continue
             for uu in range(mul_c):
                 slot_src.append((ib, uoff_of_slot[pth.slot] + uvu.group_entry_u0[e] + uu))
-        if any(sb < 0 for sb, _ in slot_src):
+        if any(sb == -1 for sb, _ in slot_src):
             return None
         K = len(slot_src)
         T = -(-K // AGG_CHUNK)
@@ -921,8 +976,10 @@
             base = np.array([flat_of.get((int(b), io), 0) for b in ib_], dtype=np.int64)
             g0 = base + u_ * S * mo + v
             valid = (ib_ >= 0) & (v < mo)
-            gather_parts.append(np.where(valid[None, :], g0[None, :] + np.arange(S)[:, None] * mo, -1))
-            scale_parts.append(np.full(slot.size, fan[io] ** -0.5, dtype=np.float32))
+            one = (ib_ == AGG_GATHER_ONE) & (u_ == v)
+            gather_parts.append(np.where(valid[None, :], g0[None, :] + np.arange(S)[:, None] * mo,
+                                         np.where(one, AGG_GATHER_ONE, -1)[None, :]))
+            scale_parts.append(np.where(one, 1.0, fan[io] ** -0.5).astype(np.float32))
             kmax = max(1, AGG_STAGE_W // mo_p)
             for k0 in range(0, d3, kmax):
                 kk = min(kmax, d3 - k0)
@@ -941,7 +998,22 @@
                                | (int(last and k == k0 + kk - 1) << 10) | (k << 12) | (ii << 20), t0, 0))
     gather = np.concatenate(gather_parts, axis=1).astype(np.int64)
     assert gather.max() < flat
+    extra = {}
+    if narrowed:
+        n = len(ent)
+        ng = np.concatenate(narrow_gather).astype(np.int64)
+        narrow_tab = np.zeros((n, TP_MAX_COMBOS), dtype=np.int64)
+        for (e, c), mo_c in narrowed.items():
+            rel = 32 * (n - e) + narrow_woff[(e, c)]
+            if rel % 4 or rel // 4 >= 1 << 15 or ent[e][8 + 12 + c] >= 1 << 16 or ent[e][8 + c] >= 1 << 20:
+                return None
+            narrow_tab[e][c] = mo_c | (narrow_woff[(e, c)] << 8)
+            ent[e][0] |= TP_KIND_NARROW
+            ent[e][8 + c] |= mo_c << 20
+            ent[e][8 + 12 + c] |= (rel // 4) << 16
+        assert 0 <= ng.min() and ng.max() < flat
+        extra = dict(narrow=narrow_tab.astype(np.int32), narrow_gather=ng, narrow_scale=np.concatenate(narrow_scale))
     return AggLinearPlan(entries=ent.astype(np.int32), ld=ld, n_chunks=chunk0,
                          io_table=np.array(io_rows, dtype=np.int32).reshape(-1, 8),
                          blocks=np.array(blocks, dtype=np.int32).reshape(-1, 4), w_stride=a_off, gather=gather,
-                         scale=np.concatenate(scale_parts), d_out=irreps_out.dim, max_mt=max_mt)
+                         scale=np.concatenate(scale_parts), d_out=irreps_out.dim, max_mt=max_mt, **extra)
```
